# lizaibeim/mmla-audio

Measured on AMD Instinct MI355X. Metric: audio clips/sec (MFCC→logits) at 1/2/4/8 MI355X; MFCC max-abs-err vs librosa, higher is better.
Workload: dtype f16x3+f32

## Files before the change

mmla_audio_amd/csrc/context.cpp:

```cpp
#include <algorithm>
#include <cstdarg>
#include <cstdio>
#include <cstdlib>

#include "internal.h"

using namespace mmla;

namespace mmla __attribute__((visibility("hidden"))) {

int fail(mmla_ctx* c, int code, const char* fmt, ...) {
  char buf[512];
  va_list ap;
  va_start(ap, fmt);
  vsnprintf(buf, sizeof(buf), fmt, ap);
  va_end(ap);
  if (c) c->err = buf;
  return code;
}

static hipEvent_t prof_event(mmla_ctx* c) {
  if (!c->prof_pool.empty()) {
    hipEvent_t e = c->prof_pool.back();
    c->prof_pool.pop_back();
    return e;
  }
  hipEvent_t e = nullptr;
  (void)hipEventCreate(&e);
  return e;
}

int prof_begin(mmla_ctx* c, int stage) {
  if (!c->prof_on) return -1;
  ProfRec r{stage, prof_event(c), prof_event(c), 0.0};
  (void)hipEventRecord(r.a, c->stream);
  c->prof_pending.push_back(r);
  return (int)c->prof_pending.size() - 1;
}

void prof_end(mmla_ctx* c, int idx, double work) {
  if (idx < 0) return;
  ProfRec& r = c->prof_pending[idx];
  r.work = work;
  (void)hipEventRecord(r.b, c->stream);
}

int prof_collect(mmla_ctx* c) {
  for (ProfRec& r : c->prof_pending) {
    HIPCHK(c, hipEventSynchronize(r.b));
    float ms = 0.0f;
    HIPCHK(c, hipEventElapsedTime(&ms, r.a, r.b));
    c->prof_ms[r.stage] += ms;
    c->prof_work[r.stage] += r.work;
    c->prof_n[r.stage] += 1;
    c->prof_pool.push_back(r.a);
    c->prof_pool.push_back(r.b);
  }
  c->prof_pending.clear();
  return MMLA_OK;
}

constexpr size_t kGuardBytes = 4u << 20;
constexpr int kGuardByte = 0xA5;

int ws_get(mmla_ctx* c, int slot, size_t bytes, void** out) {
  if ((int)c->ws.size() <= slot) {
    c->ws.resize(slot + 1, nullptr);
    c->ws_size.resize(slot + 1, 0);
    c->ws_guard.resize(slot + 1, 0);
  }
  const char* ge = std::getenv("MMLA_WS_GUARD");
  const size_t guard = ge && ge[0] == '1' ? kGuardBytes : 0;
  if (c->ws_size[slot] < bytes || (guard && c->ws_size[slot] != bytes)) {
    if (c->ws[slot]) {
      HIPCHK(c, hipStreamSynchronize(c->stream));
      HIPCHK(c, hipFree(static_cast<char*>(c->ws[slot]) - c->ws_guard[slot]));
      c->ws[slot] = nullptr;
      c->ws_size[slot] = 0;
    }
    void* p = nullptr;
    if (c->debug_fail_allocs > 0) {
      --c->debug_fail_allocs;
      return fail(c, MMLA_E_OOM, "workspace slot %d: injected allocation failure (MMLA_DEBUG_FAIL_ALLOC)", slot);
    }
    if (hipMalloc(&p, bytes + 2 * guard) != hipSuccess) {
      (void)hipGetLastError();
      return fail(c, MMLA_E_OOM, "hipMalloc(%zu) failed for workspace slot %d", bytes, slot);
    }
    if (guard) {
      HIPCHK(c, hipMemsetAsync(p, kGuardByte, guard, c->stream));
      HIPCHK(c, hipMemsetAsync(static_cast<char*>(p) + guard + bytes, kGuardByte, guard, c->stream));
    }
    const char* pe = std::getenv("MMLA_WS_POISON");
    if (pe && pe[0])
      HIPCHK(c, hipMemsetAsync(static_cast<char*>(p) + guard, (int)std::strtol(pe, nullptr, 0) & 255,
                               bytes, c->stream));
    c->ws[slot] = static_cast<char*>(p) + guard;
    c->ws_size[slot] = bytes;
    c->ws_guard[slot] = guard;
  }
  *out = c->ws[slot];
  return MMLA_OK;
}

int ws_release(mmla_ctx* c) {
  HIPCHK(c, hipStreamSynchronize(c->stream));
  for (size_t i = 0; i < c->ws.size(); ++i)
    if (c->ws[i]) {
      HIPCHK(c, hipFree(static_cast<char*>(c->ws[i]) - c->ws_guard[i]));
      c->ws[i] = nullptr;
      c->ws_size[i] = 0;
      c->ws_guard[i] = 0;
    }
  return MMLA_OK;
}

static int ws_check_guards(mmla_ctx* c) {
  std::vector<unsigned char> h(kGuardBytes);
  for (size_t slot = 0; slot < c->ws.size(); ++slot) {
    const size_t g = c->ws_guard[slot];
    if (!c->ws[slot] || !g) continue;
    for (int side = 0; side < 2; ++side) {
      const char* d = static_cast<const char*>(c->ws[slot]) + (side ? c->ws_size[slot] : -(ptrdiff_t)g);
      HIPCHK(c, hipMemcpy(h.data(), d, g, hipMemcpyDeviceToHost));
      for (size_t i = 0; i < g; ++i)
        if (h[i] != kGuardByte)
          return fail(c, MMLA_E_HIP, "workspace slot %zu: %s guard overwritten at byte %zu", slot,
                      side ? "trailing" : "leading", side ? i : g - i);
    }
  }
  return MMLA_OK;
}

int finish(mmla_ctx* c, bool dev) {
  HIPCHK(c, hipGetLastError());
  bool guarded = false;
  for (size_t g : c->ws_guard) guarded |= g != 0;
  if (!dev || guarded) HIPCHK(c, hipStreamSynchronize(c->stream));
  if (guarded) return ws_check_guards(c);
  return MMLA_OK;
}

constexpr double kOdBytesPerClip = 3.0 * 128 * 151 * 32 * 4 + 128 * 151 * 3 + 128 * 151 * 4 +
                                   19 * 128 * 4 + 512 * 4 + 64;
constexpr double kSiBytesPerClip = 4.0 * 256 * 32 * 4 + 256 * 39 * 4 + 8 * 128 * 4 + 512 * 4 +
                                   1024 * 4 + 64;

int64_t microbatch(mmla_ctx* c, bool od) {
  const int64_t user = od ? c->od_mb : c->si_mb;
  if (user > 0) return user;
  const int64_t cap = od ? c->od_mb_cap : c->si_mb_cap;
  size_t fr = 0, tot = 0;
  if (hipMemGetInfo(&fr, &tot) != hipSuccess) {
    (void)hipGetLastError();
    return cap;
  }
  double held = 0;
  for (size_t b : c->ws_size) held += (double)b;
  int64_t fit = (int64_t)(((double)fr + held) * 0.9 / (od ? kOdBytesPerClip : kSiBytesPerClip));
  fit = fit / kMinMicrobatch * kMinMicrobatch;
  return std::max(kMinMicrobatch, std::min(cap, fit));
}

}

struct EnvSwitch {
  const char* name;
  bool mmla_ctx::*no;
  int mmla_ctx::*num;
};
static const EnvSwitch kEnvSwitches[] = {
    {"MMLA_DEBUG_FAIL_ALLOC", nullptr, &mmla_ctx::debug_fail_allocs},
    {"MMLA_NO_SIU", &mmla_ctx::siu, nullptr},
    {"MMLA_NO_SIPU", &mmla_ctx::sipu, nullptr},
    {"MMLA_NO_SIFIN", &mmla_ctx::sifin, nullptr},
    {"MMLA_NO_SIPAIR", &mmla_ctx::sipair, nullptr},
    {"MMLA_NO_SICHAIN", &mmla_ctx::sichain, nullptr},
    {"MMLA_NO_LSTM_SPLIT", &mmla_ctx::lstm_split, nullptr},
    {"MMLA_LSTM_SPLIT_MAX", nullptr, &mmla_ctx::lstm_split_max},
    {"MMLA_DEBUG_LSTM_SPIN", nullptr, &mmla_ctx::lstm_spin},
    {"MMLA_NO_SIPAD", &mmla_ctx::si_pad_feat, nullptr},
    {"MMLA_NO_ODU", &mmla_ctx::odu, nullptr},
    {"MMLA_NO_ODW", &mmla_ctx::odw, nullptr},
    {"MMLA_NO_VADW", &mmla_ctx::vadw, nullptr},
    {"MMLA_VADW", nullptr, &mmla_ctx::vadw_all},
    {"MMLA_RB_TILE", &mmla_ctx::rbs, nullptr},
    {"MMLA_NO_PIN_OUT", &mmla_ctx::pin_small, nullptr},
};

extern "C" {

int mmla_abi_version(void) { return MMLA_ABI_VERSION; }

int mmla_create(int device, mmla_ctx** out) {
  if (!out) return MMLA_E_INVALID;
  *out = nullptr;
  int ndev = 0;
  if (hipGetDeviceCount(&ndev) != hipSuccess || ndev == 0) return MMLA_E_HIP;
  if (device < 0 || device >= ndev) return MMLA_E_INVALID;
  if (hipSetDevice(device) != hipSuccess) return MMLA_E_HIP;
  mmla_ctx* c = new mmla_ctx();
  c->device = device;
  for (const EnvSwitch& s : kEnvSwitches)
    if (const char* v = std::getenv(s.name)) {
      if (s.no) c->*s.no = std::atoi(v) == 0;
      else c->*s.num = std::atoi(v);
    }
  if (hipStreamCreateWithFlags(&c->own_stream, hipStreamDefault) != hipSuccess) {
    delete c;
    return MMLA_E_HIP;
  }
  c->stream = c->own_stream;
  if (hipMalloc(&c->range_dev, 4 * sizeof(int)) != hipSuccess ||
      hipMemset(c->range_dev, 0, 4 * sizeof(int)) != hipSuccess ||
      hipHostMalloc(&c->range_host, 2 * sizeof(int), hipHostMallocDefault) != hipSuccess) {
    mmla_destroy(c);
    return MMLA_E_HIP;
  }
  if (c->pin_small) {
    const unsigned fl = hipHostMallocMapped | hipHostMallocCoherent;
    if (hipHostMalloc(reinterpret_cast<void**>(&c->range_map), 64, fl) != hipSuccess ||
        hipHostGetDevicePointer(reinterpret_cast<void**>(&c->range_map_dev), c->range_map, 0) != hipSuccess ||
        hipHostMalloc(reinterpret_cast<void**>(&c->pin_out), kPinSlots * kPinSlotBytes, fl) != hipSuccess ||
        hipHostGetDevicePointer(reinterpret_cast<void**>(&c->pin_out_dev), c->pin_out, 0) != hipSuccess ||
        hipHostMalloc(reinterpret_cast<void**>(&c->pin_in), kPinInBytes, hipHostMallocDefault) != hipSuccess) {
      mmla_destroy(c);
      return MMLA_E_HIP;
    }
    c->range_map[0] = c->range_map[1] = 0;
  }
  OdFeTables ot;
  od_fe_build_tables(&ot);
  if (!od_fe_tables_ok(ot)) {
    mmla_destroy(c);
    return MMLA_E_INVALID;
  }
  SiFeTables st;
  si_fe_build_tables(&st);
  if (!si_fe_tables_ok(st)) {
    mmla_destroy(c);
    return MMLA_E_INVALID;
  }
  if (hipMalloc(&c->od_tables, sizeof(OdFeTables)) != hipSuccess ||
      hipMalloc(&c->si_tables, sizeof(SiFeTables)) != hipSuccess ||
      hipMemcpy(c->od_tables, &ot, sizeof(ot), hipMemcpyHostToDevice) != hipSuccess ||
      hipMemcpy(c->si_tables, &st, sizeof(st), hipMemcpyHostToDevice) != hipSuccess) {
    mmla_destroy(c);
    return MMLA_E_HIP;
  }
  *out = c;
  return MMLA_OK;
}

int mmla_destroy(mmla_ctx* c) {
  if (!c) return MMLA_E_INVALID;
  (void)hipSetDevice(c->device);
  if (c->stream) (void)hipStreamSynchronize(c->stream);
  free_allocs(c->od_allocs);
  free_allocs(c->si_allocs);
  free_allocs(c->si_head_allocs);
  for (size_t i = 0; i < c->ws.size(); ++i)
    if (c->ws[i]) (void)hipFree(static_cast<char*>(c->ws[i]) - c->ws_guard[i]);
  if (c->od_tables) (void)hipFree(c->od_tables);
  if (c->si_tables) (void)hipFree(c->si_tables);
  if (c->nr_tables) (void)hipFree(c->nr_tables);
  if (c->nr_thresh) (void)hipFree(c->nr_thresh);
  if (c->range_dev) (void)hipFree(c->range_dev);
  if (c->vad_state) (void)hipFree(c->vad_state);
  if (c->cap_state) (void)hipFree(c->cap_state);
  for (void* p : c->cap_buf)
    if (p) (void)hipFree(p);
  if (c->range_host) (void)hipHostFree(c->range_host);
  if (c->range_map) (void)hipHostFree(c->range_map);
  if (c->pin_out) (void)hipHostFree(c->pin_out);
  if (c->pin_in) (void)hipHostFree(c->pin_in);
  (void)prof_collect(c);
  for (hipEvent_t e : c->prof_pool) (void)hipEventDestroy(e);
  if (c->own_stream) (void)hipStreamDestroy(c->own_stream);
  delete c;
  return MMLA_OK;
}

const char* mmla_last_error(const mmla_ctx* c) { return c ? c->err.c_str() : "null context"; }

int mmla_set_stream(mmla_ctx* c, void* s) {
  if (!c) return MMLA_E_INVALID;
  hipStream_t ns = s ? static_cast<hipStream_t>(s) : c->own_stream;
  if (ns != c->stream) {
    HIPCHK(c, hipSetDevice(c->device));
    hipEvent_t e = nullptr;
    HIPCHK(c, hipEventCreateWithFlags(&e, hipEventDisableTiming));
    const hipError_t r1 = hipEventRecord(e, c->stream);
    const hipError_t r2 = r1 == hipSuccess ? hipStreamWaitEvent(ns, e, 0) : r1;
    (void)hipEventDestroy(e);
    HIPCHK(c, r2);
  }
  c->stream = ns;
  return MMLA_OK;
}

int mmla_range_check(mmla_ctx* c, int64_t* f32_reruns) {
  if (!c) return MMLA_E_INVALID;
  HIPCHK(c, hipSetDevice(c->device));
  HIPCHK(c, hipStreamSynchronize(c->stream));
  if (f32_reruns) *f32_reruns = c->range_reruns;
  int flag = 0, timeout = 0;
  HIPCHK(c, hipMemcpy(&flag, c->range_dev, sizeof(int), hipMemcpyDeviceToHost));
  HIPCHK(c, hipMemcpy(&timeout, c->range_dev + 3, sizeof(int), hipMemcpyDeviceToHost));
  if (timeout) {
    HIPCHK(c, hipMemset(c->range_dev + 3, 0, sizeof(int)));
    return fail(c, MMLA_E_HIP,
                "a device-pointer call since the last check ran the split BiLSTM and one of its "
                "workgroups timed out waiting for the others: its probabilities are NaN; re-run it");
  }
  if (flag) {
    HIPCHK(c, hipMemset(c->range_dev, 0, sizeof(int)));
    return fail(c, MMLA_E_RANGE,
                "a device-pointer call since the last check split an operand outside the fp16 "
                "range (|x| >= 65504): its results are not valid; re-run it with MMLA_PREC_F32");
  }
  return MMLA_OK;
}

int mmla_debug_counters(mmla_ctx* c, int64_t* f32_reruns, int64_t* lstm_split_reruns) {
  if (!c) return MMLA_E_INVALID;
  if (f32_reruns) *f32_reruns = c->range_reruns;
  if (lstm_split_reruns) *lstm_split_reruns = c->lstm_split_reruns;
  return MMLA_OK;
}

int mmla_synchronize(mmla_ctx* c) { return mmla_range_check(c, nullptr); }

int mmla_get_microbatch(mmla_ctx* c, int64_t* od_clips, int64_t* si_clips) {
  if (!c) return MMLA_E_INVALID;
  HIPCHK(c, hipSetDevice(c->device));
  if (od_clips) *od_clips = microbatch(c, true);
  if (si_clips) *si_clips = microbatch(c, false);
  return MMLA_OK;
}

int mmla_release_workspace(mmla_ctx* c) {
  if (!c) return MMLA_E_INVALID;
  HIPCHK(c, hipSetDevice(c->device));
  CHK(ws_release(c));
  for (int i = 0; i < 5; ++i)
    if (c->cap_buf[i]) {
      HIPCHK(c, hipFree(c->cap_buf[i]));
      c->cap_buf[i] = nullptr;
      c->cap_bytes[i] = 0;
    }
  return MMLA_OK;
}

int mmla_set_precision(mmla_ctx* c, int mode) {
  if (!c || (mode != MMLA_PREC_F32 && mode != MMLA_PREC_F16X3)) return MMLA_E_INVALID;
  c->precision = mode;
  return MMLA_OK;
}

int mmla_set_microbatch(mmla_ctx* c, int64_t od, int64_t si) {
  if (!c || od < 0 || si < 0) return MMLA_E_INVALID;
  c->od_mb = od;
  c->si_mb = si;
  c->od_mb_cap = kOdMicrobatch;
  c->si_mb_cap = kSiMicrobatch;
  return MMLA_OK;
}

int mmla_debug_ws_slot(mmla_ctx* c, int slot, void** ptr, size_t* bytes) {
  if (!c || !ptr || !bytes || slot < 0) return MMLA_E_INVALID;
  const bool have = slot < (int)c->ws.size() && c->ws[slot];
  *ptr = have ? c->ws[slot] : nullptr;
  *bytes = have ? c->ws_size[slot] : 0;
  return MMLA_OK;
}

int mmla_profile_enable(mmla_ctx* c, int on) {
  if (!c) return MMLA_E_INVALID;
  c->prof_on = on != 0;
  return MMLA_OK;
}

int mmla_profile_read(mmla_ctx* c, double* ms, int64_t* launches, double* work, int reset) {
  if (!c) return MMLA_E_INVALID;
  CHK(prof_collect(c));
  for (int i = 0; i < MMLA_NSTAGES; ++i) {
    if (ms) ms[i] = c->prof_ms[i];
    if (launches) launches[i] = c->prof_n[i];
    if (work) work[i] = c->prof_work[i];
    if (reset) {
      c->prof_ms[i] = 0.0;
      c->prof_n[i] = 0;
      c->prof_work[i] = 0.0;
    }
  }
  return MMLA_OK;
}

}
```

mmla_audio_amd/csrc/internal.h:

```cpp
#pragma once
#include <hip/hip_runtime.h>

#include <cstdint>
#include <cstring>
#include <string>
#include <vector>

#include "../../include/mmla.h"
#include "nr.h"
#include "od_fe.h"
#include "si_fe.h"
#include "ssim.h"
#include "vad.h"

namespace mmla __attribute__((visibility("hidden"))) {

constexpr int OD_H = 128, OD_W = 151, OD_PIX = OD_H * OD_W;
constexpr int OD_IMG = OD_PIX * 3;
constexpr int SI_T = 256, SI_D = 39;
constexpr int SI_NEED_SAMPLES = 160 * 259 + 400;
constexpr int CH[9] = {32, 32, 32, 64, 64, 64, 128, 128, 128};
constexpr bool POOL[9] = {true, false, false, true, false, false, true, false, false};

struct ConvW {
  float* wt = nullptr;
  float* bias = nullptr;
  uint16_t* wh = nullptr;
  uint16_t* wl = nullptr;
  uint16_t* fh = nullptr;
  uint16_t* fl = nullptr;
  int kh = 0, kw = 0, cin = 0, cout = 0, cout_pad = 0, cin_pad = 0, kpad = 0;
  float wscale = 256.0f;
  float unscale() const { return 1.0f / (16.0f * wscale); }
};
struct BnW {
  float* scale = nullptr;
  float* shift = nullptr;
  int c = 0;
};
struct LstmW {
  float* wcat[2] = {nullptr, nullptr};
  float* bias[2] = {nullptr, nullptr};
  uint16_t* wth[2] = {nullptr, nullptr};
  uint16_t* wtl[2] = {nullptr, nullptr};
  float ws[2] = {256.0f, 256.0f};
};
struct ResUnitW {
  BnW bn_in, bn_mid;
  ConvW ca, cb, sc;
};
struct OdNet {
  ConvW stem;
  ResUnitW blk[9];
  LstmW lstm;
  float* head_w = nullptr;
  float* head_b = nullptr;
};
struct SiNet {
  ConvW stem;
  ResUnitW unit[9];
  BnW final_bn;
  LstmW lstm;
  ConvW dense;
  int k = 0, head = 0;
};

struct ProfRec {
  int stage;
  hipEvent_t a, b;
  double work;
};

constexpr int64_t kOdMicrobatch = 16384;
constexpr int64_t kSiMicrobatch = 65536;
constexpr int64_t kMinMicrobatch = 64;

constexpr size_t kPinSlotBytes = 64u << 10;
constexpr size_t kPinInBytes = 1u << 20;
constexpr int kPinSlots = 4;

}

struct mmla_ctx {
  bool prof_on = false;
  std::vector<mmla::ProfRec> prof_pending;
  std::vector<hipEvent_t> prof_pool;
  double prof_ms[MMLA_NSTAGES] = {0};
  double prof_work[MMLA_NSTAGES] = {0};
  int64_t prof_n[MMLA_NSTAGES] = {0};
  int device = 0;
  hipStream_t stream = nullptr;
  hipStream_t own_stream = nullptr;
  std::string err;
  OdFeTables* od_tables = nullptr;
  SiFeTables* si_tables = nullptr;
  bool od_loaded = false, si_loaded = false;
  mmla::OdNet od;
  mmla::SiNet si;
  std::vector<void*> od_allocs, si_allocs;
  std::vector<void*> si_head_allocs;
  std::vector<void*> ws;
  std::vector<size_t> ws_size;
  std::vector<size_t> ws_guard;
  int64_t od_mb = 0, si_mb = 0;
  int64_t od_mb_cap = mmla::kOdMicrobatch, si_mb_cap = mmla::kSiMicrobatch;
  int debug_fail_allocs = 0;
  int precision = MMLA_PREC_F16X3;
  bool siu = true;
  bool sipu = true;
  bool sifin = true;
  bool sipair = true;
  bool sichain = true;
  bool si_pad_feat = true;
  bool odu = true;
  bool odw = true;
  bool vadw = true;
  int vadw_all = 0;
  bool rbs = true;
  bool lstm_split = true;
  int lstm_split_max = 128;
  int lstm_spin = 0;
  int* range_dev = nullptr;
  int* range_host = nullptr;
  bool pin_small = true;
  int* range_map = nullptr;
  int* range_map_dev = nullptr;
  char* pin_out = nullptr;
  char* pin_out_dev = nullptr;
  char* pin_in = nullptr;
  int* range_ptr = nullptr;
  int* timeout_ptr = nullptr;
  int64_t lstm_split_reruns = 0;
  int64_t range_reruns = 0;
  bool od_f32_only = false, si_f32_only = false;
  bool loading_f16_bad = false;
  bool si_base_f16_bad = false;
  VadState* vad_state = nullptr;
  int64_t vad_streams = 0;
  int32_t* cap_state = nullptr;
  int cap_cur = 0;
  int64_t cap_streams = 0;
  int32_t cap_rate = 0, cap_channels = 0, cap_channel = 0, cap_ir = 0, cap_or = 0;
  void* cap_buf[5] = {nullptr, nullptr, nullptr, nullptr, nullptr};
  size_t cap_bytes[5] = {0, 0, 0, 0, 0};
  NrTables* nr_tables = nullptr;
  float* nr_thresh = nullptr;
  int64_t nr_profiles = 0;
  bool nr_ready = false;
  int32_t nr_bank_sr = 0;
  double ns_time_constant_s = 2.0, ns_thresh_n_mult = 2.0, ns_sigmoid_slope = 10.0;
  int32_t ns_sr = 16000;
};

namespace mmla __attribute__((visibility("hidden"))) {

int fail(mmla_ctx* c, int code, const char* fmt, ...);

#define HIPCHK(ctx, expr)                                                                        \
  do {                                                                                           \
    hipError_t e_ = (expr);                                                                      \
    if (e_ != hipSuccess)                                                                        \
      return mmla::fail(ctx, MMLA_E_HIP, "%s failed: %s (%s:%d)", #expr, hipGetErrorString(e_), \
                        __FILE__, __LINE__);                                                     \
  } while (0)

#define CHK(expr)              \
  do {                         \
    int r_ = (expr);           \
    if (r_ != MMLA_OK) return r_; \
  } while (0)

int prof_begin(mmla_ctx* c, int stage);
void prof_end(mmla_ctx* c, int idx, double work);
int prof_collect(mmla_ctx* c);

#define LAUNCH(c, st, wk, expr)                  \
  do {                                           \
    const int pi_ = mmla::prof_begin((c), (st)); \
    HIPCHK((c), (expr));                         \
    mmla::prof_end((c), pi_, (wk));              \
  } while (0)

enum Slot {
  S_PCM = 0, S_LENS, S_IMG, S_X, S_T1, S_T2, S_T3, S_SEQ, S_HOUT, S_LOGIT, S_FEAT, S_SILENT,
  S_OUT0, S_OUT1, S_OUT2, S_OUT3, S_IN,
  S_NR_S, S_NR_BITS, S_NR_FMAX, S_NR_FRAMES, S_NR_ITEMS, S_NR_Y, S_NR_ROWS,
  S_VAD_SPEECH, S_VAD_OUT, S_VAD_LENS, S_RS_TR, S_RS_WIN, S_LSTM,
  S_TRAIN,
  S_IMG2, S_GATE_Y0, S_GATE_Y1, S_SSIM,
  S_NR_PROF, S_COND_Q, S_COND_KEPT,
  S_ROOM_P, S_ROOM_A,
  S_ENROL_VAD, S_ENROL_NW
};

enum CapBuf { CB_RAW = 0, CB_FRAMES, CB_ITEM, CB_OUT, CB_LENS };

int ws_get(mmla_ctx* c, int slot, size_t bytes, void** out);
int ws_release(mmla_ctx* c);
int64_t microbatch(mmla_ctx* c, bool od);
int finish(mmla_ctx* c, bool dev);
void free_allocs(std::vector<void*>& al);
inline bool vad_use_wave(const mmla_ctx* c, int64_t n_streams) {
  return c->vadw && (c->vadw_all > 0 || vad_wave_streams(n_streams));
}
int nr_reduce_dev(mmla_ctx* c, const float* y, int64_t n_signals, int64_t stride, int64_t len, float* out,
                  const int32_t* profile = nullptr, bool nonstationary = false);

template <typename T>
int in_ptr(mmla_ctx* c, const T* user, size_t count, bool dev, int slot, const T** d) {
  *d = user;
  if (dev || !user) return MMLA_OK;
  void* p = nullptr;
  CHK(ws_get(c, slot, count * sizeof(T), &p));
  HIPCHK(c, hipMemcpyAsync(p, user, count * sizeof(T), hipMemcpyHostToDevice, c->stream));
  *d = static_cast<const T*>(p);
  return MMLA_OK;
}

template <typename T>
int out_ptr(mmla_ctx* c, T* user, int64_t off, size_t count, bool dev, int slot, T** d) {
  if (!user) {
    *d = nullptr;
    return MMLA_OK;
  }
  if (dev) {
    *d = user + off;
    return MMLA_OK;
  }
  if (c->pin_small && c->pin_out_dev && slot >= S_OUT0 && slot < S_OUT0 + kPinSlots &&
      count * sizeof(T) <= kPinSlotBytes) {
    *d = reinterpret_cast<T*>(c->pin_out_dev + (size_t)(slot - S_OUT0) * kPinSlotBytes);
    return MMLA_OK;
  }
  void* p = nullptr;
  CHK(ws_get(c, slot, count * sizeof(T), &p));
  *d = static_cast<T*>(p);
  return MMLA_OK;
}

template <typename T>
int copy_back(mmla_ctx* c, T* user, int64_t off, const T* d, size_t count, bool dev) {
  if (!user || dev) return MMLA_OK;
  const char* dc = reinterpret_cast<const char*>(d);
  if (c->pin_out_dev && dc >= c->pin_out_dev && dc < c->pin_out_dev + kPinSlots * kPinSlotBytes) {
    HIPCHK(c, hipStreamSynchronize(c->stream));
    std::memcpy(user + off, c->pin_out + (dc - c->pin_out_dev), count * sizeof(T));
    return MMLA_OK;
  }
  HIPCHK(c, hipMemcpyAsync(user + off, d, count * sizeof(T), hipMemcpyDeviceToHost, c->stream));
  return MMLA_OK;
}


struct OdGate {
  const int32_t* lens = nullptr;
  int clip_len = -1;
  uint8_t* silent = nullptr;
  const float* ssim = nullptr;
  float ssim_threshold = 0.0f;
};

int run_od_net(mmla_ctx* c, const uint8_t* img_u8, const float* img_f32, int64_t n, float* probs,
               int32_t* argmax, OdGate gate = OdGate(), int stop = -1, const float** tap = nullptr,
               int64_t* tap_n = nullptr);
int run_si_net(mmla_ctx* c, const float* x, int64_t n, float* probs, int32_t* argmax,
               const uint8_t* silent, int ldx = SI_D, const float** tap = nullptr);

}
```

mmla_audio_amd/csrc/net_runners.cpp:

```cpp
#include <algorithm>

#include "conv.h"
#include "conv_h3.h"
#include "internal.h"
#include "nets.h"
#include "odu.h"
#include "resblk.h"
#include "siu.h"

using namespace mmla;

namespace {

ConvArgs conv_args(const ConvW& w, const float* x, float* y, int n, int h, int wd, int stride,
                   const BnW* bn, int pro, int epi, const float* res) {
  ConvArgs a{};
  a.x = x;
  a.wt = w.wt;
  a.bias = w.bias;
  a.scale = bn ? bn->scale : nullptr;
  a.shift = bn ? bn->shift : nullptr;
  a.res = res;
  a.y = y;
  a.n = n;
  a.h = h;
  a.w = wd;
  a.cin = w.cin;
  a.ho = (h + stride - 1) / stride;
  a.wo = (wd + stride - 1) / stride;
  a.cout = w.cout;
  a.cout_pad = w.cout_pad;
  a.ldy = w.cout;
  a.kh = w.kh;
  a.kw = w.kw;
  a.stride = stride;
  const int th = std::max((a.ho - 1) * stride + w.kh - h, 0);
  const int tw = std::max((a.wo - 1) * stride + w.kw - wd, 0);
  a.pad_h = th / 2;
  a.pad_w = tw / 2;
  a.pro = pro;
  a.epi = epi;
  return a;
}

double conv_flops(const ConvArgs& a) {
  return 2.0 * (double)a.n * a.ho * a.wo * a.kh * a.kw * a.cin * a.cout;
}

int conv_run(mmla_ctx* c, const ConvArgs& a, int stage = MMLA_STAGE_CONV) {
  LAUNCH(c, stage, conv_flops(a), conv_launch(a, c->stream));
  return MMLA_OK;
}

ConvH3Args conv_h3_args(const ConvW& w, const float* x, float* y, int n, int h, int wd, const BnW* bn,
                        int pro, int epi, const float* res, int* range_flag) {
  ConvH3Args a{};
  a.x = x;
  a.wh = w.wh;
  a.wl = w.wl;
  a.unscale = w.unscale();
  a.bias = w.bias;
  a.scale = bn ? bn->scale : nullptr;
  a.shift = bn ? bn->shift : nullptr;
  a.res = res;
  a.y = y;
  a.n = n;
  a.h = h;
  a.w = wd;
  a.cin = w.cin;
  a.cin_pad = w.cin_pad;
  a.cout = w.cout;
  a.cout_pad = w.cout_pad;
  a.kh = w.kh;
  a.kw = w.kw;
  a.pad_h = (w.kh - 1) / 2;
  a.pad_w = (w.kw - 1) / 2;
  a.pro = pro;
  a.epi = epi;
  a.range_flag = range_flag;
  return a;
}

int conv_spatial(mmla_ctx* c, const ConvW& w, const float* x, float* y, int n, int h, int wd,
                 const BnW* bn, int pro, int epi, const float* res, bool pool_out = false,
                 int pool_in_h = 0, const ConvW* sc = nullptr, const float* sc_x = nullptr,
                 int sc_h = 0) {
  if (c->precision == MMLA_PREC_F16X3 && w.wh) {
    ConvH3Args a = conv_h3_args(w, x, y, n, h, wd, bn, pro, epi, res, c->range_ptr);
    double sc_flops = 0.0;
    if (sc && sc_x) {
      a.sc_x = sc_x;
      a.sc_wh = sc->wh;
      a.sc_wl = sc->wl;
      a.sc_bias = sc->bias;
      a.sc_cin = sc->cin;
      a.sc_h = sc_h;
      a.sc_unscale = sc->unscale();
      sc_flops = sc_h > 0 ? 2.0 * n * h * sc->cin * sc->cout
                          : 2.0 * n * ((h + 1) / 2) * ((wd + 1) / 2) * sc->cin * sc->cout;
    }
    a.pool_in = pool_in_h > 0;
    a.h_in = pool_in_h;
    a.pool_out = pool_out ? 1 : 0;
    LAUNCH(c, MMLA_STAGE_CONV, 2.0 * n * h * wd * w.kh * w.kw * w.cin * w.cout + sc_flops,
           conv_h3_launch(a, c->stream));
    return MMLA_OK;
  }
  ConvArgs a = conv_args(w, x, y, n, h, wd, 1, bn, pro, epi, res);
  if (!pool_out) return conv_run(c, a);
  return fail(c, MMLA_E_INVALID, "pooled epilogue needs the 3xFP16 conv path");
}

int ws_floats(mmla_ctx* c, int slot, size_t count, float** out) {
  void* p = nullptr;
  CHK(ws_get(c, slot, count * sizeof(float), &p));
  *out = static_cast<float*>(p);
  return MMLA_OK;
}

double lstm_flops(int64_t n, int T, int D) { return 2.0 * n * T * 2 * (256.0 + D) * 1024.0; }

hipError_t lstm_run(mmla_ctx* c, const LstmW& L, const float* seq, int64_t n, int T, float* out) {
  if (c->precision == MMLA_PREC_F16X3 && L.wth[0] && c->lstm_split &&
      n <= std::min(c->lstm_split_max, bilstm_h3_split_max_clips())) {
    void* ws = nullptr;
    if (ws_get(c, S_LSTM, bilstm_h3_split_ws_bytes(), &ws) != MMLA_OK) return hipErrorOutOfMemory;
    return bilstm_h3_split_launch(seq, (int)n, T, 128, L.wth[0], L.wtl[0], L.wth[1], L.wtl[1],
                                  L.bias[0], L.bias[1], out, c->range_ptr, L.ws[0], L.ws[1], ws,
                                  c->timeout_ptr, c->lstm_spin, c->stream);
  }
  if (c->precision == MMLA_PREC_F16X3 && L.wth[0])
    return bilstm_h3_launch(seq, (int)n, T, 128, L.wth[0], L.wtl[0], L.wth[1], L.wtl[1], L.bias[0],
                            L.bias[1], out, c->range_ptr, L.ws[0], L.ws[1], c->stream);
  return bilstm_launch(seq, (int)n, T, 128, L.wcat[0], L.wcat[1], L.bias[0], L.bias[1], out,
                       c->stream);
}


enum OdPath {
  OD_STRIPS,
  OD_TILES,
  OD_ODU,
  OD_PAIR
};
struct OdChoice {
  OdPath path;
  bool stem;
  int strips;
};

bool strips_ok(const ResUnitW& B, bool pool, int h, int w) {
  return B.ca.wh && B.cb.wh && (!pool || B.sc.wh) && B.ca.cin_pad == B.ca.cin && B.ca.cout_pad == 32 &&
         B.cb.cin_pad == 32 && B.cb.cout_pad == 32 && B.cb.kh == 4 && B.cb.kw == 1 &&
         (!pool || (B.sc.cin_pad == B.ca.cin && B.sc.cout_pad == 32)) &&
         rbs_supported(h, w, B.ca.cin, B.ca.cout, pool);
}

bool tiles_ok(const ResUnitW& B, bool pool) {
  return B.ca.fh && B.cb.fh && B.cb.kpad == 4 * B.cb.cin && (!pool || B.sc.fh) &&
         resblk_supported(B.ca.cin, B.ca.cout, pool);
}

bool odu_ok(const ResUnitW& B, bool pool, int h, int w) {
  return B.ca.wh && B.cb.wh && (!pool || B.sc.wh) && odu_supported(h, w, B.ca.cin, B.ca.cout, pool) &&
         B.ca.cin_pad == B.ca.cin && B.ca.cout_pad == B.ca.cout && B.cb.cin == B.ca.cout &&
         B.cb.cout == B.ca.cout && B.cb.cin_pad == B.cb.cin && B.cb.cout_pad == B.cb.cout &&
         B.cb.kh == 4 && B.cb.kw == 1 &&
         (!pool || (B.sc.cin == B.ca.cin && B.sc.cout == B.ca.cout && B.sc.cout_pad == B.sc.cout));
}

OdChoice od_choose(const mmla_ctx* c, const ResUnitW& B, int b, int h, int w, int stop) {
  OdChoice k{OD_PAIR, false, 1};
  if (c->precision != MMLA_PREC_F16X3) return k;
  if (c->rbs && strips_ok(B, POOL[b], h, w)) k.path = OD_STRIPS;
  else if (tiles_ok(B, POOL[b])) k.path = OD_TILES;
  else if (c->odu && odu_ok(B, POOL[b], h, w)) {
    k.path = OD_ODU;
    k.strips = c->odw && odu_two_strips(h, w, B.ca.cin, B.ca.cout, POOL[b]) ? 2 : 1;
  }
  k.stem = b == 0 && stop != 0 && (k.path == OD_STRIPS || k.path == OD_TILES);
  return k;
}

ResBlkArgs resblk_args(const ResUnitW& B, bool pool, bool fused, const float* x, float* y, int64_t n,
                       int h, int w, int* range_flag, const ConvW* stem, const uint8_t* img_u8,
                       const float* img_f32) {
  ResBlkArgs r{};
  r.x = x;
  r.y = y;
  r.w1h = fused ? B.ca.fh : B.ca.wh;
  r.w1l = fused ? B.ca.fl : B.ca.wl;
  r.b1 = B.ca.bias;
  r.u1 = B.ca.unscale();
  r.s1 = B.bn_in.scale;
  r.t1 = B.bn_in.shift;
  r.w2h = fused ? B.cb.fh : B.cb.wh;
  r.w2l = fused ? B.cb.fl : B.cb.wl;
  r.b2 = B.cb.bias;
  r.u2 = B.cb.unscale();
  r.s2 = B.bn_mid.scale;
  r.t2 = B.bn_mid.shift;
  if (pool) {
    r.wsh = fused ? B.sc.fh : B.sc.wh;
    r.wsl = fused ? B.sc.fl : B.sc.wl;
    r.bs = B.sc.bias;
    r.us = B.sc.unscale();
  }
  if (stem) {
    r.x = nullptr;
    r.img8 = img_u8;
    r.imgf = img_u8 ? nullptr : img_f32;
    r.wst = stem->wt;
    r.bst = stem->bias;
    r.ldst = stem->cout_pad;
  }
  r.n = (int)n;
  r.h = h;
  r.w = w;
  r.range_flag = range_flag;
  return r;
}

OduArgs odu_args(const ResUnitW& B, bool pool, const float* x, float* y, int64_t n, int* range_flag) {
  OduArgs o{};
  o.x = x;
  o.y = y;
  o.wah = B.ca.wh;
  o.wal = B.ca.wl;
  o.wbh = B.cb.wh;
  o.wbl = B.cb.wl;
  o.ba = B.ca.bias;
  o.bb = B.cb.bias;
  o.s_in = B.bn_in.scale;
  o.t_in = B.bn_in.shift;
  o.s_mid = B.bn_mid.scale;
  o.t_mid = B.bn_mid.shift;
  o.ua = B.ca.unscale();
  o.ub = B.cb.unscale();
  o.n = (int)n;
  o.range_flag = range_flag;
  if (pool) {
    o.wsh = B.sc.wh;
    o.wsl = B.sc.wl;
    o.bs = B.sc.bias;
    o.us = B.sc.unscale();
  }
  return o;
}

double od_block_flops(const ResUnitW& B, bool pool, int64_t n, int h, int w) {
  return 2.0 * n * h * w * (9.0 * B.ca.cin * B.ca.cout + 4.0 * B.cb.cin * B.cb.cout) +
         (pool ? 2.0 * n * ((h + 1) / 2) * ((w + 1) / 2) * B.sc.cin * B.sc.cout : 0.0);
}

int od_block_pair(mmla_ctx* c, const ResUnitW& B, bool pool, int n, int h, int w, float* X, float*& T1,
                  float*& T2, float** out) {
  CHK(conv_spatial(c, B.ca, X, T1, n, h, w, &B.bn_in, PRO_BN_ELU, EPI_BIAS, nullptr));
  if (!pool) {
    *out = X;
    return conv_spatial(c, B.cb, T1, X, n, h, w, &B.bn_mid, PRO_BN_ELU, EPI_ADD, X);
  }
  if (c->precision != MMLA_PREC_F16X3) {
    CHK(conv_spatial(c, B.cb, T1, T2, n, h, w, &B.bn_mid, PRO_BN_ELU, EPI_BIAS, nullptr));
    ConvArgs s = conv_args(B.sc, X, T1, n, h, w, 2, nullptr, PRO_NONE, EPI_ADD_POOL, T2);
    s.hp = h;
    s.wp = w;
    CHK(conv_run(c, s));
  } else if (B.sc.wh && B.sc.cout == B.cb.cout && B.cb.cout_pad == B.sc.cout_pad) {
    CHK(conv_spatial(c, B.cb, T1, T2, n, h, w, &B.bn_mid, PRO_BN_ELU, EPI_BIAS, nullptr, true, 0, &B.sc,
                     X));
    std::swap(T1, T2);
  } else {
    CHK(conv_spatial(c, B.cb, T1, T2, n, h, w, &B.bn_mid, PRO_BN_ELU, EPI_BIAS, nullptr, true));
    CHK(conv_run(c, conv_args(B.sc, X, T1, n, h, w, 2, nullptr, PRO_NONE, EPI_ADD, T2)));
  }
  *out = T1;
  return MMLA_OK;
}

}

namespace mmla __attribute__((visibility("hidden"))) {

int run_od_net(mmla_ctx* c, const uint8_t* img_u8, const float* img_f32, int64_t n, float* probs,
               int32_t* argmax, OdGate gate, int stop, const float** tap, int64_t* tap_n) {
  const OdNet& W = c->od;
  const size_t big = (size_t)n * OD_PIX * 32;
  float *X, *T1, *T2, *SEQ, *H;
  CHK(ws_floats(c, S_X, big, &X));
  CHK(ws_floats(c, S_T1, big, &T1));
  CHK(ws_floats(c, S_T2, big, &T2));
  CHK(ws_floats(c, S_SEQ, (size_t)n * 19 * 128, &SEQ));
  CHK(ws_floats(c, S_HOUT, (size_t)n * 512, &H));
  const double stem_flops = 2.0 * n * OD_PIX * 3 * 16;
  const OdChoice first = od_choose(c, W.blk[0], 0, OD_H, OD_W, stop);
  if (!first.stem)
    LAUNCH(c, MMLA_STAGE_GLUE, stem_flops,
           od_stem_launch(img_u8, img_f32, n * OD_PIX, W.stem.cout_pad, W.stem.wt, W.stem.bias, X,
                          c->stream));
  int h = OD_H, w = OD_W;
  if (stop == 0) {
    *tap = X;
    *tap_n = n * OD_PIX * 16;
    return MMLA_OK;
  }
  for (int b = 0; b < 9; ++b) {
    const ResUnitW& B = W.blk[b];
    const bool pool = POOL[b];
    const OdChoice k = b == 0 ? first : od_choose(c, B, b, h, w, stop);
    const double flops = od_block_flops(B, pool, n, h, w) + (k.stem ? stem_flops : 0.0);
    float* out = T1;
    switch (k.path) {
      case OD_STRIPS:
      case OD_TILES: {
        const bool tiles = k.path == OD_TILES;
        const ResBlkArgs r = resblk_args(B, pool, tiles, X, T1, n, h, w, c->range_ptr,
                                         k.stem ? &W.stem : nullptr, img_u8, img_f32);
        LAUNCH(c, MMLA_STAGE_CONV, flops,
               tiles ? resblk_launch(r, B.ca.cin, B.ca.cout, pool, c->stream)
                     : rbs_launch(r, B.ca.cin, B.ca.cout, pool, c->stream));
        break;
      }
      case OD_ODU: {
        const OduArgs o = odu_args(B, pool, X, T1, n, c->range_ptr);
        LAUNCH(c, MMLA_STAGE_CONV, flops,
               odu_launch(o, h, w, B.ca.cin, B.ca.cout, pool, k.strips, c->stream));
        break;
      }
      case OD_PAIR:
        CHK(od_block_pair(c, B, pool, (int)n, h, w, X, T1, T2, &out));
        break;
    }
    if (pool) {
      h = (h + 1) / 2;
      w = (w + 1) / 2;
    }
    if (out != X) std::swap(X, T1);
    if (stop == b + 1) {
      *tap = X;
      *tap_n = n * h * w * CH[b];
      return MMLA_OK;
    }
  }
  LAUNCH(c, MMLA_STAGE_GLUE, (double)n * h * w * 128,
         mean_h_launch(X, (int)n, h, w, 128, SEQ, c->stream));
  if (stop == 10) {
    *tap = SEQ;
    *tap_n = n * w * 128;
    return MMLA_OK;
  }
  LAUNCH(c, MMLA_STAGE_LSTM, lstm_flops(n, w, 128),
         lstm_run(c, W.lstm, SEQ, n, w, H));
  if (stop == 11) {
    *tap = H;
    *tap_n = n * 512;
    return MMLA_OK;
  }
  LAUNCH(c, MMLA_STAGE_HEAD, 2.0 * n * 512 * 2,
         od_head_launch(H, (int)n, W.head_w, W.head_b, probs, argmax,
                        gate.lens, gate.clip_len, gate.silent, gate.ssim, gate.ssim_threshold,
                        c->stream));
  return MMLA_OK;
}

}


namespace {

bool siu_ok(const ResUnitW& U, int cin) {
  return U.ca.wh && U.cb.wh && siu_chain_supported(cin, cin, false, 1, false) && U.ca.cin == cin &&
         U.ca.cout == cin && U.cb.cin == cin && U.cb.cout == cin && U.ca.cin_pad == cin && U.ca.cout_pad == cin &&
         U.cb.cout_pad == cin;
}

bool sipu_ok(const ResUnitW& U, int cin) {
  return U.ca.wh && U.cb.wh && U.sc.wh && siu_chain_supported(cin, U.ca.cout, true, 1, false) &&
         U.ca.cin_pad == cin && U.ca.cout_pad == U.ca.cout && U.cb.cin == U.ca.cout && U.cb.cout == U.ca.cout &&
         U.cb.cout_pad == U.ca.cout && U.sc.cin == cin && U.sc.cout == U.ca.cout &&
         U.sc.cout_pad == U.ca.cout;
}

int si_choose(const mmla_ctx* c, const SiNet& W, int u) {
  if (!c->siu || c->precision != MMLA_PREC_F16X3) return 0;
  const int cin = W.unit[u].ca.cin, C = W.unit[u].ca.cout;
  auto plain = [&](int v) { return v < 9 && !POOL[v] && siu_ok(W.unit[v], C); };
  if (POOL[u]) {
    if (!c->sipu || !sipu_ok(W.unit[u], cin)) return 0;
    return c->sichain && siu_chain_supported(cin, C, true, 3, false) && plain(u + 1) && plain(u + 2) ? 3 : 1;
  }
  if (!siu_ok(W.unit[u], cin)) return 0;
  return c->sipair && siu_chain_supported(cin, cin, false, 2, false) && plain(u + 1) ? 2 : 1;
}

double si_unit_flops(const ResUnitW& U, bool pool, int64_t n, int t) {
  return 2.0 * n * t *
         (3.0 * U.ca.cin * U.ca.cout + 3.0 * U.cb.cin * U.cb.cout + (pool ? 1.0 * U.sc.cin * U.sc.cout : 0.0));
}

SiuArgs siu_args(const ResUnitW& U, const float* x, float* y, int64_t n, int t, int* range_flag,
                 int t_src = 0) {
  SiuArgs s{};
  s.n = (int)n;
  s.t = t;
  s.range_flag = range_flag;
  s.x = x;
  s.y = y;
  s.wah = U.ca.wh;
  s.wal = U.ca.wl;
  s.wbh = U.cb.wh;
  s.wbl = U.cb.wl;
  s.ba = U.ca.bias;
  s.bb = U.cb.bias;
  s.s_in = U.bn_in.scale;
  s.t_in = U.bn_in.shift;
  s.s_mid = U.bn_mid.scale;
  s.t_mid = U.bn_mid.shift;
  s.ua = U.ca.unscale();
  s.ub = U.cb.unscale();
  if (t_src > 0) {
    s.t_src = t_src;
    s.wsh = U.sc.wh;
    s.wsl = U.sc.wl;
    s.bs = U.sc.bias;
    s.us = U.sc.unscale();
  }
  return s;
}

}

namespace mmla __attribute__((visibility("hidden"))) {

int run_si_net(mmla_ctx* c, const float* x, int64_t n, float* probs, int32_t* argmax,
               const uint8_t* silent, int ldx, const float** tap) {
  const SiNet& W = c->si;
  const size_t big = (size_t)n * SI_T * 32;
  float *X, *T1, *XP, *R, *SEQ, *H, *L;
  CHK(ws_floats(c, S_X, big, &X));
  CHK(ws_floats(c, S_T1, big, &T1));
  CHK(ws_floats(c, S_T2, big, &XP));
  CHK(ws_floats(c, S_T3, big, &R));
  CHK(ws_floats(c, S_SEQ, (size_t)n * 8 * 128, &SEQ));
  CHK(ws_floats(c, S_HOUT, (size_t)n * 512, &H));
  CHK(ws_floats(c, S_LOGIT, (size_t)n * W.dense.cout_pad, &L));
  int t = SI_T;
  const bool h3 = c->precision == MMLA_PREC_F16X3;
  bool fused_final = false;
  ConvW stem = W.stem;
  if (ldx == SI_D + 1 && h3 && stem.wh && stem.cin_pad > SI_D) stem.cin = ldx;
  else if (ldx != SI_D) return fail(c, MMLA_E_INVALID, "padded SI features need the 3xFP16 stem");
  CHK(conv_spatial(c, stem, x, X, (int)n, t, 1, nullptr, PRO_NONE, EPI_BIAS, nullptr));
  for (int u = 0; u < 9; ++u) {
    const ResUnitW& U = W.unit[u];
    const int cin = U.ca.cin;
    const bool pool = POOL[u];
    const int tp = pool ? (t + 1) / 2 : t;
    const int units = si_choose(c, W, u);
    float* out = R;
    if (units > 0) {
      const int C = U.ca.cout;
      SiuArgs s[3];
      double flops = 0.0;
      for (int k = 0; k < units; ++k) {
        const bool first = k == 0;
        s[k] = siu_args(W.unit[u + k], first ? X : nullptr, k == units - 1 ? R : nullptr, n, tp, c->range_ptr,
                        first && pool ? t : 0);
        flops += si_unit_flops(W.unit[u + k], first && pool, n, tp);
      }
      if (u + units == 9 && c->sifin && tp % 4 == 0 && siu_chain_supported(cin, C, pool, units, true)) {
        SiuArgs& last = s[units - 1];
        last.y = nullptr;
        last.seq = SEQ;
        last.fs = W.final_bn.scale;
        last.ft = W.final_bn.shift;
        fused_final = true;
      }
      LAUNCH(c, MMLA_STAGE_CONV, flops, siu_chain_launch(s, units, pool, cin, C, c->stream));
      u += units - 1;
    } else if (pool) {
      if (h3 && U.ca.wh) {
        CHK(conv_spatial(c, U.ca, X, T1, (int)n, tp, 1, &U.bn_in, PRO_BN_RELU, EPI_BIAS, nullptr,
                         false, t));
      } else {
        LAUNCH(c, MMLA_STAGE_GLUE, (double)n * t * cin,
               maxpool_t2_launch(X, (int)n, t, cin, XP, c->stream));
        CHK(conv_spatial(c, U.ca, XP, T1, (int)n, tp, 1, &U.bn_in, PRO_BN_RELU, EPI_BIAS, nullptr));
      }
      if (h3 && U.cb.wh && U.sc.wh && U.sc.cout == U.cb.cout && U.sc.cout_pad == U.cb.cout_pad) {
        CHK(conv_spatial(c, U.cb, T1, R, (int)n, tp, 1, &U.bn_mid, PRO_BN_RELU, EPI_ADD, nullptr, false,
                         0, &U.sc, X, t));
      } else {
        CHK(conv_run(c, conv_args(U.sc, X, R, (int)n, t, 1, 2, nullptr, PRO_NONE, EPI_BIAS, nullptr)));
        CHK(conv_spatial(c, U.cb, T1, R, (int)n, tp, 1, &U.bn_mid, PRO_BN_RELU, EPI_ADD, R));
      }
    } else {
      CHK(conv_spatial(c, U.ca, X, T1, (int)n, t, 1, &U.bn_in, PRO_BN_RELU, EPI_BIAS, nullptr));
      CHK(conv_spatial(c, U.cb, T1, X, (int)n, t, 1, &U.bn_mid, PRO_BN_RELU, EPI_ADD, X));
      out = X;
    }
    if (out != X) std::swap(X, R);
    t = tp;
  }
  if (!fused_final)
    LAUNCH(c, MMLA_STAGE_GLUE, 3.0 * n * t * 128,
           bn_relu_avgpool4_launch(X, (int)n, t, 128, W.final_bn.scale, W.final_bn.shift,
                                   SEQ, c->stream));
  LAUNCH(c, MMLA_STAGE_LSTM, lstm_flops(n, t / 4, 128),
         lstm_run(c, W.lstm, SEQ, n, t / 4, H));
  if (tap) {
    *tap = H;
    return MMLA_OK;
  }
  if (h3 && W.dense.wh && W.dense.cin % 32 == 0) {
    ConvH3Args a = conv_h3_args(W.dense, H, L, (int)n, 1, 1, nullptr, PRO_NONE, EPI_BIAS, nullptr,
                                c->range_ptr);
    a.cout = W.dense.cout_pad;
    LAUNCH(c, MMLA_STAGE_HEAD, 2.0 * n * W.dense.cin * W.dense.cout, conv_h3_launch(a, c->stream));
  } else {
    ConvArgs d = conv_args(W.dense, H, L, (int)n, 1, 1, 1,
                           nullptr, PRO_NONE, EPI_BIAS, nullptr);
    d.ldy = W.dense.cout_pad;
    CHK(conv_run(c, d, MMLA_STAGE_HEAD));
  }
  LAUNCH(c, MMLA_STAGE_HEAD, 4.0 * n * W.k,
         si_head_launch(L, (int)n, W.k, W.dense.cout_pad, W.head, probs,
                        argmax, silent, c->stream));
  return MMLA_OK;
}

}
```

mmla_audio_amd/csrc/rbs.hip:

```cpp
#include "f16x3.h"
#include "resblk.h"

namespace {

constexpr int NT = 256;
constexpr int TW = 16;
constexpr int R = 8;
constexpr int C = 32;
#ifndef RBS_TRACE
#define RBS_TRACE 0
#endif
#if RBS_TRACE
__device__ unsigned long long rbs_trace_buf[2048 * 4 * 4 * 8];
#define RBS_T(i) do { if (bid < 2048 && k >= 2 && k < 6) tt[i] = __builtin_amdgcn_s_memtime(); } while (0)
#define RBS_TFLUSH() do { if (bid < 2048 && k >= 2 && k < 6 && lane == 0) { for (int i_ = 0; i_ < 8; ++i_) rbs_trace_buf[(((size_t)bid * 4 + wave) * 4 + (k - 2)) * 8 + i_] = tt[i_]; } } while (0)
#else
#define RBS_T(i) do { } while (0)
#define RBS_TFLUSH() do { } while (0)
#endif

template <int H, int W, int CIN, bool POOL>
struct SG {
  static constexpr int XW = TW + 2;
  static constexpr int XRING = R + 2, TRING = R + 3;
  static constexpr int XROW = XW * CIN;
  static constexpr int XPLANE = XRING * XROW;
  static constexpr int TROW = TW * C;
  static constexpr int TPLANE = TRING * TROW;
  static constexpr int NCHUNK = H / R;
  static constexpr int STRIPS = (W + TW - 1) / TW;
  static constexpr int QPP = CIN / 4;
  static constexpr int MAXT = (R * XW * QPP + NT - 1) / NT;
  static constexpr int MAXT0 = (4 * XW * QPP + NT - 1) / NT;
  static constexpr int KPT = CIN / 16;
  static constexpr int KS1 = 9 * KPT, KS2 = 8;
  static constexpr bool W2L = CIN == 16;
  static constexpr int MINB = CIN == 16 ? 3 : 2;
  static constexpr int PF = 3;
  static constexpr int PD = CIN == 16 ? 1 : 2;
  static_assert(H % R == 0, "geometry");
  static_assert(NT % QPP == 0, "a thread's channel quad is fixed");
  static_assert(XROW <= 1024 && W * CIN * 4 < 65536 && W * 12 < 65536, "staging task fields");
};

template <int CIN>
MMLA_DEV int xoff(int slot, int x, int g) {
  constexpr int XROW = (TW + 2) * CIN;
  const int f = CIN == 32 ? ((x >> 1) & 3) : ((x >> 1) & 1);
  return slot * XROW + x * CIN + 8 * (g ^ f);
}
template <bool POOL>
MMLA_DEV int toff(int slot, int j, int c, int g) {
  const int f = POOL ? (((c >> 2) ^ (2 * (j & 1))) & 3) : ((c >> 2) & 3);
  return slot * (TW * C) + c * C + 8 * (g ^ f);
}

template <int H, int W, int CIN, bool POOL, bool STEM>
__global__ void __launch_bounds__(NT, (SG<H, W, CIN, POOL>::MINB)) rbs_kernel(ResBlkArgs a) {
  using G = SG<H, W, CIN, POOL>;
  static_assert(!STEM || (CIN == 16 && POOL), "the stem feeds block 1");
  static_assert(POOL || CIN == C, "residual blocks keep their width");
  __shared__ __attribute__((aligned(16))) _Float16 sx[2 * G::XPLANE];
  __shared__ __attribute__((aligned(16))) _Float16 st[2 * G::TPLANE];
  __shared__ float4 spar[3 * C / 4 + (STEM ? 16 : 0)];
  __shared__ __attribute__((aligned(16))) _Float16 sw2[G::W2L ? 2 * G::KS2 * 512 : 8];

  const int tid = threadIdx.x, lane = tid & 63;
  const int wave = __builtin_amdgcn_readfirstlane(tid >> 6);
  const int h = lane >> 5;
  const uint32_t bid = xcd_block_id();
  const int clip = (int)(bid / G::STRIPS);
  const int w0 = (int)(bid - (uint32_t)clip * G::STRIPS) * TW;
  const int lofs = lane * 8;
  float rmax = 0.0f;

  float* const sp = reinterpret_cast<float*>(spar);
  if (tid < C) {
    const float s2 = a.s2[tid];
    sp[tid] = 16.0f * (s2 * a.u1);
    sp[C + tid] = 16.0f * fmaf(a.b1[tid], s2, a.t2[tid]);
    sp[2 * C + tid] = a.b2[tid];
  }
  if constexpr (STEM) {
    if (tid < 64) {
      const int co = tid >> 2, k = tid & 3;
      sp[3 * C + tid] = k < 3 ? a.wst[k * a.ldst + co] : a.bst[co];
    }
  }
  const __amdgpu_buffer_rsrc_t rw1h = w_rsrc(a.w1h), rw1l = w_rsrc(a.w1l);
  f16x8 w2h[G::W2L ? 1 : G::KS2], w2l[G::W2L ? 1 : G::KS2];
  if constexpr (G::W2L) {
    for (int e = tid; e < 2 * G::KS2 * 64; e += NT) {
      const int pl = e / (G::KS2 * 64), i = e - pl * (G::KS2 * 64);
      *reinterpret_cast<f16x8*>(sw2 + 8 * e) = *reinterpret_cast<const f16x8*>((pl ? a.w2l : a.w2h) + 8 * i);
    }
  } else {
    const __amdgpu_buffer_rsrc_t rw2h = w_rsrc(a.w2h), rw2l = w_rsrc(a.w2l);
#pragma unroll
    for (int s = 0; s < G::KS2; ++s) {
      w2h[s] = w_frag(rw2h, s * 512, lofs);
      w2l[s] = w_frag(rw2l, s * 512, lofs);
    }
  }
  f16x8 wsh_, wsl_;
  if constexpr (POOL) {
    wsh_ = w_frag(w_rsrc(a.wsh), 0, lofs);
    wsl_ = w_frag(w_rsrc(a.wsl), 0, lofs);
  }
  const int q = tid % G::QPP;
  float bnw[4][4];
  __syncthreads();
#pragma unroll
  for (int c = 0; c < 4; ++c) {
    const float s16 = 16.0f * a.s1[4 * q + c], t16 = 16.0f * a.t1[4 * q + c];
    if constexpr (STEM) {
      const float4 v = spar[3 * C / 4 + 4 * q + c];
      bnw[c][0] = s16 * v.x;
      bnw[c][1] = s16 * v.y;
      bnw[c][2] = s16 * v.z;
      bnw[c][3] = fmaf(s16, v.w, t16);
    } else {
      bnw[c][0] = s16;
      bnw[c][1] = t16;
    }
  }

  constexpr uint32_t ROWB = STEM ? 0u : (uint32_t)W * CIN * 4;
  const __amdgpu_buffer_rsrc_t rx = STEM ? w_rsrc(nullptr) :
      __builtin_amdgcn_make_buffer_rsrc(const_cast<float*>(a.x) + (int64_t)clip * H * W * CIN, (short)0,
                                        (int)(H * ROWB), 0x00020000);
  const bool im8 = STEM && a.img8 != nullptr;
  const __amdgpu_buffer_rsrc_t rimg = !STEM ? w_rsrc(nullptr) :
      __builtin_amdgcn_make_buffer_rsrc(im8 ? (void*)(a.img8 + (int64_t)clip * H * W * 3)
                                            : (void*)(a.imgf + (int64_t)clip * H * W * 3),
                                        (short)0, (int)(H * W * 3 * (im8 ? 1 : 4)), 0x00020000);
  uint32_t tinfo[G::MAXT];
#pragma unroll
  for (int j = 0; j < G::MAXT; ++j) {
    const int t = tid + j * NT;
    const int px = t / G::QPP;
    const int rr = px / G::XW, x = px - rr * G::XW;
    const int iw = w0 - 1 + x;
    const bool col_ok = iw >= 0 && iw < W;
    const uint32_t tc = !col_ok ? 0u : STEM ? (uint32_t)iw * (a.img8 ? 3u : 12u) : (uint32_t)(iw * CIN + 4 * q) * 4u;
    tinfo[j] = (uint32_t)(xoff<CIN>(0, x, q >> 1) + 4 * (q & 1)) | ((uint32_t)(rr & 15) << 10) |
               ((uint32_t)col_ok << 14) | ((uint32_t)(rr < R) << 15) | (tc << 16);
  }
  auto load_src = [&](int ih, int iw, bool col_ok) -> float4 {
    if constexpr (STEM) {
      const int pix = ih * W + iw;
      const bool ok = col_ok && ih >= 0 && ih < H;
      if (im8) {
        const uint32_t off = ok ? (uint32_t)pix * 3u : 0x80000000u;
        const uint32_t r = __builtin_amdgcn_raw_buffer_load_b8(rimg, off, 0, 0);
        const uint32_t g = __builtin_amdgcn_raw_buffer_load_b8(rimg, off + 1u, 0, 0);
        const uint32_t b = __builtin_amdgcn_raw_buffer_load_b8(rimg, off + 2u, 0, 0);
        return make_float4(__builtin_bit_cast(float, r), __builtin_bit_cast(float, g), __builtin_bit_cast(float, b), 0.f);
      }
      const uint32_t off = ok ? (uint32_t)pix * 12u : 0x80000000u;
      return make_float4(__builtin_bit_cast(float, __builtin_amdgcn_raw_buffer_load_b32(rimg, off, 0, 0)),
                         __builtin_bit_cast(float, __builtin_amdgcn_raw_buffer_load_b32(rimg, off + 4u, 0, 0)),
                         __builtin_bit_cast(float, __builtin_amdgcn_raw_buffer_load_b32(rimg, off + 8u, 0, 0)), 0.f);
    } else {
      const uint32_t off = col_ok ? (uint32_t)ih * ROWB + (uint32_t)(iw * CIN + 4 * q) * 4u : 0x80000000u;
      return __builtin_bit_cast(float4, __builtin_amdgcn_raw_buffer_load_b128(rx, off, 0, 0));
    }
  };
  auto img_px = [&](float4 v) -> float4 {
    if (im8)
      return make_float4((float)__builtin_bit_cast(uint32_t, v.x), (float)__builtin_bit_cast(uint32_t, v.y),
                         (float)__builtin_bit_cast(uint32_t, v.z), 0.f);
    return v;
  };
  auto load_task = [&](int r0, int j) -> float4 {
    const uint32_t ti = tinfo[j];
    const uint32_t off = (ti >> 14) & 1u ? (uint32_t)((r0 + (int)((ti >> 10) & 15)) * (STEM ? W * 3 * (im8 ? 1 : 4) : (int)ROWB)) + (ti >> 16)
                                         : 0x80000000u;
    if constexpr (STEM) {
      if (im8) {
        const uint32_t r = __builtin_amdgcn_raw_buffer_load_b8(rimg, off, 0, 0);
        const uint32_t g = __builtin_amdgcn_raw_buffer_load_b8(rimg, off + 1u, 0, 0);
        const uint32_t b = __builtin_amdgcn_raw_buffer_load_b8(rimg, off + 2u, 0, 0);
        return make_float4(__builtin_bit_cast(float, r), __builtin_bit_cast(float, g), __builtin_bit_cast(float, b), 0.f);
      }
      return make_float4(__builtin_bit_cast(float, __builtin_amdgcn_raw_buffer_load_b32(rimg, off, 0, 0)),
                         __builtin_bit_cast(float, __builtin_amdgcn_raw_buffer_load_b32(rimg, off + 4u, 0, 0)),
                         __builtin_bit_cast(float, __builtin_amdgcn_raw_buffer_load_b32(rimg, off + 8u, 0, 0)), 0.f);
    } else {
      return __builtin_bit_cast(float4, __builtin_amdgcn_raw_buffer_load_b128(rx, off, 0, 0));
    }
  };
  auto stage4 = [&](int o, bool in, float4 v, auto MASK_) {
    constexpr bool MASK = decltype(MASK_)::value;
    if constexpr (STEM) v = img_px(v);
    float u[4];
#pragma unroll
    for (int c = 0; c < 4; ++c) {
      if constexpr (STEM) {
        float acc = v.x * bnw[c][0];
        acc = fmaf(v.y, bnw[c][1], acc);
        acc = fmaf(v.z, bnw[c][2], acc);
        u[c] = acc + bnw[c][3];
      } else {
        u[c] = fmaf((&v.x)[c], bnw[c][0], bnw[c][1]);
      }
    }
    float e[4];
#pragma unroll
    for (int c = 0; c < 4; ++c) e[c] = (!MASK || in) ? elu16(u[c]) : 0.0f;
    rmax = fmaxf(rmax, amax4(e[0], e[1], e[2], e[3]));
    f16x4 hv, lv;
    split4(e[0], e[1], e[2], e[3], hv, lv);
    *reinterpret_cast<f16x4*>(sx + o) = hv;
    *reinterpret_cast<f16x4*>(sx + G::XPLANE + o) = lv;
  };
  auto stage_task = [&](int r0, int j, float4 v, auto MASK_) {
    const uint32_t ti = tinfo[j];
    if (((ti >> 14) & 3u) != 3u) return;
    const int rr = (int)((ti >> 10) & 15);
    uint32_t slot = (uint32_t)((r0 + 1) % G::XRING) + (uint32_t)rr;
    slot = min(slot, slot - (uint32_t)G::XRING);
    stage4((int)slot * G::XROW + (int)(ti & 1023), r0 + rr < H, v, MASK_);
  };
  for (int e = tid; e < 2 * G::XRING * G::XW * G::QPP; e += NT) {
    const int pl = e / (G::XRING * G::XW * G::QPP), r = e - pl * (G::XRING * G::XW * G::QPP);
    const int slot = r / (G::XW * G::QPP), x = (r / G::QPP) % G::XW, qq = r % G::QPP;
    const int iw = w0 - 1 + x;
    if (iw < 0 || iw >= W)
      *reinterpret_cast<f16x4*>(sx + pl * G::XPLANE + xoff<CIN>(slot, x, qq >> 1) + 4 * (qq & 1)) = f16x4{};
  }
  const int n = lane & 31, nr = n >> 4, nc = n & 15;
  int xco[3][G::KPT];
#pragma unroll
  for (int dx = 0; dx < 3; ++dx)
#pragma unroll
    for (int ks = 0; ks < G::KPT; ++ks) xco[dx][ks] = xoff<CIN>(0, nc + dx, G::KPT == 2 ? 2 * ks + h : h);

  f16x8 w1h[G::PF], w1l[G::PF];
  auto gemm1_issue = [&]() {
#pragma unroll
    for (int s = 0; s < G::PF; ++s) {
      w1h[s] = w_frag(rw1h, s * 512, lofs);
      w1l[s] = w_frag(rw1l, s * 512, lofs);
    }
  };
  auto gemm1 = [&](int j0) -> f32x16 {
    f32x16 acc;
#pragma unroll
    for (int i = 0; i < 16; ++i) acc[i] = 0.0f;
    int xr[3];
#pragma unroll
    for (int dy = 0; dy < 3; ++dy) {
      const uint32_t sl = (uint32_t)(j0 % G::XRING) + (uint32_t)(nr + dy);
      xr[dy] = (int)min(sl, sl - (uint32_t)G::XRING) * G::XROW;
    }
    auto xo = [&](int s) {
      const int tap = s / G::KPT, ks = s % G::KPT;
      return xr[tap / 3] + xco[tap % 3][ks];
    };
    f16x8 nxh = *reinterpret_cast<const f16x8*>(sx + xo(0));
    f16x8 nxl = *reinterpret_cast<const f16x8*>(sx + G::XPLANE + xo(0));
#pragma unroll
    for (int s = 0; s < G::KS1; ++s) {
      const f16x8 bh = w1h[s % G::PF], bl = w1l[s % G::PF];
      if (s + G::PF < G::KS1) {
        w1h[s % G::PF] = w_frag(rw1h, (s + G::PF) * 512, lofs);
        w1l[s % G::PF] = w_frag(rw1l, (s + G::PF) * 512, lofs);
      }
      const f16x8 xh = nxh, xl = nxl;
      if (s + 1 < G::KS1) {
        nxh = *reinterpret_cast<const f16x8*>(sx + xo(s + 1));
        nxl = *reinterpret_cast<const f16x8*>(sx + G::XPLANE + xo(s + 1));
      }
      acc = __builtin_amdgcn_mfma_f32_32x32x16_f16(bl, xh, acc, 0, 0, 0);
      acc = __builtin_amdgcn_mfma_f32_32x32x16_f16(bh, xl, acc, 0, 0, 0);
      acc = __builtin_amdgcn_mfma_f32_32x32x16_f16(bh, xh, acc, 0, 0, 0);
      __builtin_amdgcn_sched_barrier(0);
    }
    return acc;
  };
  auto t1_write = [&](int j0, const f32x16& acc) {
    const int j = j0 + nr;
    const uint32_t sl = (uint32_t)((j0 + 1) % G::TRING) + (uint32_t)nr;
    const int slot = (int)min(sl, sl - (uint32_t)G::TRING);
    if (j0 < H) {
#pragma unroll
      for (int jj = 0; jj < 4; ++jj) {
        const int c0 = 8 * jj + 4 * h;
        const float4 sv = spar[c0 / 4], cv = spar[C / 4 + c0 / 4];
        float e[4];
        e[0] = elu16(fmaf(acc[4 * jj + 0], sv.x, cv.x));
        e[1] = elu16(fmaf(acc[4 * jj + 1], sv.y, cv.y));
        e[2] = elu16(fmaf(acc[4 * jj + 2], sv.z, cv.z));
        e[3] = elu16(fmaf(acc[4 * jj + 3], sv.w, cv.w));
        rmax = fmaxf(rmax, amax4(e[0], e[1], e[2], e[3]));
        f16x4 hv, lv;
        split4(e[0], e[1], e[2], e[3], hv, lv);
        const int o = toff<POOL>(slot, j, nc, jj) + 4 * h;
        *reinterpret_cast<f16x4*>(st + o) = hv;
        *reinterpret_cast<f16x4*>(st + G::TPLANE + o) = lv;
      }
    } else {
#pragma unroll
      for (int jj = 0; jj < 4; ++jj) {
        const int o = toff<POOL>(slot, j, nc, jj) + 4 * h;
        *reinterpret_cast<f16x4*>(st + o) = f16x4{};
        *reinterpret_cast<f16x4*>(st + G::TPLANE + o) = f16x4{};
      }
    }
  };

  {
    constexpr int T0 = 4 * G::XW * G::QPP;
#pragma unroll
    for (int j = 0; j < G::MAXT0; ++j) {
      const int t = tid + j * NT;
      const int px = t / G::QPP;
      const int rr = px / G::XW, x = px - rr * G::XW;
      const int ih = rr - 1, iw = w0 - 1 + x;
      const bool col_ok = iw >= 0 && iw < W;
      const float4 v = load_src(ih, iw, col_ok);
      if (t < T0 && col_ok)
        stage4(xoff<CIN>((ih + 1) % G::XRING, x, q >> 1) + 4 * (q & 1), ih >= 0, v, std::true_type{});
    }
    for (int e = tid; e < 2 * G::TROW / 8; e += NT)
      *reinterpret_cast<f16x8*>(st + (e >= G::TROW / 8 ? G::TPLANE - G::TROW : 0) + 8 * e) = f16x8{};
  }
  __syncthreads();
  if (wave == 0) {
    gemm1_issue();
    const f32x16 acc = gemm1(0);
    t1_write(0, acc);
  }
  float4 preA[G::MAXT], preB[G::PD == 2 ? G::MAXT : 1];
#pragma unroll
  for (int j = 0; j < G::MAXT; ++j) preA[j] = load_task(3, j);
  if constexpr (G::PD == 2) {
#pragma unroll
    for (int j = 0; j < G::MAXT; ++j) preB[j] = load_task(3 + R, j);
  }
  __syncthreads();

  const int win = n >> 2;
  const int sc_col = w0 + 2 * win;
  float bsc = 0.0f;
  if constexpr (POOL) bsc = a.bs[n];

#if RBS_TRACE
  unsigned long long tt[8];
#endif
  static_assert(G::NCHUNK % 2 == 0, "chunk pairs");
  auto chunk = [&](const int k, float4* pre) {
    RBS_T(0);
    const int rx0 = R * k + 3;
    const int j0 = R * k + 2 + 2 * wave;
    const int o0 = R * k + 2 * wave;
    if (k + 1 < G::NCHUNK) {
#pragma unroll
      for (int j = 0; j < G::MAXT; ++j) stage_task(rx0, j, pre[j], std::false_type{});
    } else {
#pragma unroll
      for (int j = 0; j < G::MAXT; ++j) stage_task(rx0, j, pre[j], std::true_type{});
    }
    gemm1_issue();
    RBS_T(1);
    __syncthreads();
    RBS_T(2);
    {
      const f32x16 acc = gemm1(j0);
      RBS_T(3);
      t1_write(j0, acc);
    }
    RBS_T(4);
    const int pr = POOL ? (n & 3) >> 1 : nr;
    const int pc = POOL ? 2 * (n >> 2) + (n & 1) : nc;
    float4 rsd[POOL ? 1 : 4];
    float4 scpx = make_float4(0.f, 0.f, 0.f, 0.f);
    if constexpr (!POOL) {
      const uint32_t off = w0 + pc < W ? (uint32_t)(o0 + pr) * ROWB + (uint32_t)((w0 + pc) * C + 4 * h) * 4u : 0x80000000u;
#pragma unroll
      for (int jj = 0; jj < 4; ++jj)
        rsd[jj] = __builtin_bit_cast(float4, __builtin_amdgcn_raw_buffer_load_b128(rx, off, jj * 32, 0));
    } else {
      scpx = load_src(o0, sc_col, sc_col < W);
    }
    if (k + G::PD < G::NCHUNK) {
#pragma unroll
      for (int j = 0; j < G::MAXT; ++j) pre[j] = load_task(rx0 + G::PD * R, j);
    }
    __syncthreads();
    RBS_T(5);
    f32x16 acc;
#pragma unroll
    for (int i = 0; i < 16; ++i) acc[i] = 0.0f;
    {
      int tr[4], tj[4];
#pragma unroll
      for (int dy = 0; dy < 4; ++dy) {
        tj[dy] = o0 + pr - 1 + dy;
        const uint32_t sl = (uint32_t)(o0 % G::TRING) + (uint32_t)(pr + dy);
        tr[dy] = (int)min(sl, sl - (uint32_t)G::TRING);
      }
      auto to = [&](int s) { return toff<POOL>(tr[s >> 1], tj[s >> 1], pc, 2 * (s & 1) + h); };
      auto step2 = [&](f16x8 xh, f16x8 xl, f16x8 gh, f16x8 gl) {
        if constexpr (POOL) {
          acc = __builtin_amdgcn_mfma_f32_32x32x16_f16(xh, gl, acc, 0, 0, 0);
          acc = __builtin_amdgcn_mfma_f32_32x32x16_f16(xl, gh, acc, 0, 0, 0);
          acc = __builtin_amdgcn_mfma_f32_32x32x16_f16(xh, gh, acc, 0, 0, 0);
        } else {
          acc = __builtin_amdgcn_mfma_f32_32x32x16_f16(gl, xh, acc, 0, 0, 0);
          acc = __builtin_amdgcn_mfma_f32_32x32x16_f16(gh, xl, acc, 0, 0, 0);
          acc = __builtin_amdgcn_mfma_f32_32x32x16_f16(gh, xh, acc, 0, 0, 0);
        }
      };
      if constexpr (G::W2L) {
        f16x8 fxh[2], fxl[2], fgh[2], fgl[2];
        auto fetch = [&](int s) {
          fxh[s & 1] = *reinterpret_cast<const f16x8*>(st + to(s));
          fxl[s & 1] = *reinterpret_cast<const f16x8*>(st + G::TPLANE + to(s));
          fgh[s & 1] = *reinterpret_cast<const f16x8*>(sw2 + s * 512 + lofs);
          fgl[s & 1] = *reinterpret_cast<const f16x8*>(sw2 + (G::KS2 + s) * 512 + lofs);
        };
        fetch(0);
#pragma unroll
        for (int s = 0; s < G::KS2; ++s) {
          if (s + 1 < G::KS2) fetch(s + 1);
          step2(fxh[s & 1], fxl[s & 1], fgh[s & 1], fgl[s & 1]);
          if (s + 1 < G::KS2) pin_group<1, 4>(); else pin_group<1, 0>();
        }
      } else {
        f16x8 nxh = *reinterpret_cast<const f16x8*>(st + to(0));
        f16x8 nxl = *reinterpret_cast<const f16x8*>(st + G::TPLANE + to(0));
#pragma unroll
        for (int s = 0; s < G::KS2; ++s) {
          const f16x8 xh = nxh, xl = nxl;
          if (s + 1 < G::KS2) {
            nxh = *reinterpret_cast<const f16x8*>(st + to(s + 1));
            nxl = *reinterpret_cast<const f16x8*>(st + G::TPLANE + to(s + 1));
          }
          step2(xh, xl, w2h[s], w2l[s]);
          __builtin_amdgcn_sched_barrier(0);
        }
      }
    }
    RBS_T(6);
    if constexpr (!POOL) {
      const int ow = w0 + pc, oh = o0 + pr;
      if (ow < W) {
#pragma unroll
        for (int jj = 0; jj < 4; ++jj) {
          const int c0 = 8 * jj + 4 * h;
          const float4 b = spar[2 * C / 4 + c0 / 4];
          const float4 r = rsd[jj];
          const float4 v = make_float4(fmaf(acc[4 * jj + 0], a.u2, b.x) + r.x, fmaf(acc[4 * jj + 1], a.u2, b.y) + r.y,
                                       fmaf(acc[4 * jj + 2], a.u2, b.z) + r.z, fmaf(acc[4 * jj + 3], a.u2, b.w) + r.w);
          *reinterpret_cast<float4*>(a.y + (((int64_t)clip * H + oh) * W + ow) * C + c0) = v;
        }
      }
    } else {
      f32x16 sacc;
#pragma unroll
      for (int i = 0; i < 16; ++i) sacc[i] = 0.0f;
      {
        float o8[8];
        const float4 px = img_px(scpx);
#pragma unroll
        for (int c = 0; c < 8; ++c) {
          const float4 wv = spar[3 * C / 4 + 8 * h + c];
          float s = px.x * wv.x;
          s = fmaf(px.y, wv.y, s);
          s = fmaf(px.z, wv.z, s);
          o8[c] = sc_col < W ? 16.0f * (s + wv.w) : 0.0f;
        }
        rmax = fmaxf(rmax, fmaxf(amax4(o8[0], o8[1], o8[2], o8[3]), amax4(o8[4], o8[5], o8[6], o8[7])));
        f16x4 h0, l0, h1, l1;
        split4(o8[0], o8[1], o8[2], o8[3], h0, l0);
        split4(o8[4], o8[5], o8[6], o8[7], h1, l1);
        const f16x8 ah = {h0[0], h0[1], h0[2], h0[3], h1[0], h1[1], h1[2], h1[3]};
        const f16x8 al = {l0[0], l0[1], l0[2], l0[3], l1[0], l1[1], l1[2], l1[3]};
        sacc = __builtin_amdgcn_mfma_f32_32x32x16_f16(ah, wsl_, sacc, 0, 0, 0);
        sacc = __builtin_amdgcn_mfma_f32_32x32x16_f16(al, wsh_, sacc, 0, 0, 0);
        sacc = __builtin_amdgcn_mfma_f32_32x32x16_f16(ah, wsh_, sacc, 0, 0, 0);
      }
      constexpr int HP = H / 2, WP = (W + 1) / 2;
      const int co = n;
      const float b2 = sp[2 * C + co], bs = bsc;
      const int prow = (R / 2) * k + wave;
#pragma unroll
      for (int jj = 0; jj < 4; ++jj) {
        const int wdw = 2 * jj + h;
        const int cc = w0 + 2 * wdw;
        if (cc >= W) continue;
        float m0 = fmaf(acc[4 * jj + 0], a.u2, b2);
        float m1 = fmaf(acc[4 * jj + 1], a.u2, b2);
        float m2 = fmaf(acc[4 * jj + 2], a.u2, b2);
        float m3 = fmaf(acc[4 * jj + 3], a.u2, b2);
        if (cc + 1 >= W) {
          m1 = m0;
          m3 = m2;
        }
        const float mx = fmaxf(fmaxf(m0, m1), fmaxf(m2, m3)) + fmaf(sacc[4 * jj], a.us, bs);
        a.y[(((int64_t)clip * HP + prow) * WP + (w0 >> 1) + wdw) * C + co] = mx;
      }
    }
    RBS_T(7);
    RBS_TFLUSH();
  };
  if constexpr (G::PD == 2) {
#pragma unroll 1
    for (int k = 0; k < G::NCHUNK; k += 2) {
      chunk(k, preA);
      chunk(k + 1, preB);
    }
  } else {
#pragma unroll 1
    for (int k = 0; k < G::NCHUNK; ++k) chunk(k, preA);
  }
  if (!(rmax < SPLIT_MAX) && a.range_flag) *a.range_flag = 1;
}

template <int H, int W, int CIN, bool POOL, bool STEM>
hipError_t launch(const ResBlkArgs& a, hipStream_t s) {
  using G = SG<H, W, CIN, POOL>;
  const int64_t blocks = (int64_t)a.n * G::STRIPS;
  if (blocks > 0x7fffffffLL) return hipErrorInvalidValue;
  hipLaunchKernelGGL((rbs_kernel<H, W, CIN, POOL, STEM>), dim3((unsigned)blocks), dim3(NT), 0, s, a);
  return hipGetLastError();
}

}

#if RBS_TRACE
extern "C" int mmla_debug_rbs_trace(unsigned long long* out) {
  return hipMemcpyFromSymbol(out, HIP_SYMBOL(rbs_trace_buf), sizeof(rbs_trace_buf)) == hipSuccess ? 0 : -2;
}
#endif

bool rbs_supported(int h, int w, int cin, int c, bool pool) {
  return c == 32 && ((h == 128 && w == 151 && cin == 16 && pool) || (h == 64 && w == 76 && cin == 32 && !pool));
}

hipError_t rbs_launch(const ResBlkArgs& a, int cin, int c, bool pool, hipStream_t s) {
  if (a.n == 0) return hipSuccess;
  if (!rbs_supported(a.h, a.w, cin, c, pool) || !a.y || !a.w1h || !a.w1l || !a.w2h || !a.w2l)
    return hipErrorInvalidValue;
  if (pool) {
    if (!a.wsh || !a.wsl || !a.bs) return hipErrorInvalidValue;
    if (a.img8 || a.imgf) return launch<128, 151, 16, true, true>(a, s);
    return hipErrorInvalidValue;
  }
  if (!a.x || a.x == a.y) return hipErrorInvalidValue;
  return launch<64, 76, 32, false, false>(a, s);
}
```

mmla_audio_amd/csrc/resblk.h:

```cpp
#pragma once
#include <hip/hip_runtime.h>
#include <stdint.h>

struct ResBlkArgs {
  const float* x;
  const uint16_t* w1h;
  const uint16_t* w1l;
  const float* b1;
  const float* s1;
  const float* t1;
  const uint16_t* w2h;
  const uint16_t* w2l;
  const float* b2;
  const float* s2;
  const float* t2;
  const uint16_t* wsh;
  const uint16_t* wsl;
  const float* bs;
  const uint8_t* img8;
  const float* imgf;
  const float* wst;
  const float* bst;
  int ldst;
  float* y;
  int n, h, w;
  int tiles_h, tiles_w;
  int* range_flag;
  float u1, u2, us;
};

int resblk_k1pad(int cin);
bool resblk_supported(int cin, int c, bool pool);
hipError_t resblk_launch(ResBlkArgs a, int cin, int c, bool pool, hipStream_t stream);
void resblk_split_weights(const float* w, int taps, int cin, int cout, int kpad, uint16_t* hi,
                          uint16_t* lo, bool frag, float wscale);

bool rbs_supported(int h, int w, int cin, int c, bool pool);
hipError_t rbs_launch(const ResBlkArgs& a, int cin, int c, bool pool, hipStream_t stream);
```

Baseline: 169,500.

## Add LDS-staged first-conv weight variant of strip resblock kernel

```diff
diff --git a/mmla_audio_amd/csrc/context.cpp b/mmla_audio_amd/csrc/context.cpp
--- a/mmla_audio_amd/csrc/context.cpp
+++ b/mmla_audio_amd/csrc/context.cpp
@@ -185,6 +185,7 @@
     {"MMLA_NO_VADW", &mmla_ctx::vadw, nullptr},
     {"MMLA_VADW", nullptr, &mmla_ctx::vadw_all},
     {"MMLA_RB_TILE", &mmla_ctx::rbs, nullptr},
+    {"MMLA_NO_RBS_W1L", &mmla_ctx::rbs_w1l, nullptr},
     {"MMLA_NO_PIN_OUT", &mmla_ctx::pin_small, nullptr},
 };
 
diff --git a/mmla_audio_amd/csrc/internal.h b/mmla_audio_amd/csrc/internal.h
--- a/mmla_audio_amd/csrc/internal.h
+++ b/mmla_audio_amd/csrc/internal.h
@@ -117,6 +117,7 @@
   bool vadw = true;
   int vadw_all = 0;
   bool rbs = true;
+  bool rbs_w1l = true;
   bool lstm_split = true;
   int lstm_split_max = 128;
   int lstm_spin = 0;
diff --git a/mmla_audio_amd/csrc/net_runners.cpp b/mmla_audio_amd/csrc/net_runners.cpp
--- a/mmla_audio_amd/csrc/net_runners.cpp
+++ b/mmla_audio_amd/csrc/net_runners.cpp
@@ -147,6 +147,7 @@
   OdPath path;
   bool stem;
   int strips;
+  bool w1_lds;
 };
 
 bool strips_ok(const ResUnitW& B, bool pool, int h, int w) {
@@ -170,11 +171,14 @@
 }
 
 OdChoice od_choose(const mmla_ctx* c, const ResUnitW& B, int b, int h, int w, int stop) {
-  OdChoice k{OD_PAIR, false, 1};
+  OdChoice k{OD_PAIR, false, 1, false};
   if (c->precision != MMLA_PREC_F16X3) return k;
-  if (c->rbs && strips_ok(B, POOL[b], h, w)) k.path = OD_STRIPS;
-  else if (tiles_ok(B, POOL[b])) k.path = OD_TILES;
-  else if (c->odu && odu_ok(B, POOL[b], h, w)) {
+  if (c->rbs && strips_ok(B, POOL[b], h, w)) {
+    k.path = OD_STRIPS;
+    k.w1_lds = c->rbs_w1l && !POOL[b];
+  } else if (tiles_ok(B, POOL[b])) {
+    k.path = OD_TILES;
+  } else if (c->odu && odu_ok(B, POOL[b], h, w)) {
     k.path = OD_ODU;
     k.strips = c->odw && odu_two_strips(h, w, B.ca.cin, B.ca.cout, POOL[b]) ? 2 : 1;
   }
@@ -318,7 +322,7 @@
                                          k.stem ? &W.stem : nullptr, img_u8, img_f32);
         LAUNCH(c, MMLA_STAGE_CONV, flops,
                tiles ? resblk_launch(r, B.ca.cin, B.ca.cout, pool, c->stream)
-                     : rbs_launch(r, B.ca.cin, B.ca.cout, pool, c->stream));
+                     : rbs_launch(r, B.ca.cin, B.ca.cout, pool, k.w1_lds, c->stream));
         break;
       }
       case OD_ODU: {
diff --git a/mmla_audio_amd/csrc/rbs.hip b/mmla_audio_amd/csrc/rbs.hip
--- a/mmla_audio_amd/csrc/rbs.hip
+++ b/mmla_audio_amd/csrc/rbs.hip
@@ -1,523 +1,8 @@
-#include "f16x3.h"
-#include "resblk.h"
+#define RBS_KERNEL rbs_kernel
+#define RBS_W1L false
+#include "rbs_body.h"
 
 namespace {
-
-constexpr int NT = 256;
-constexpr int TW = 16;
-constexpr int R = 8;
-constexpr int C = 32;
-#ifndef RBS_TRACE
-#define RBS_TRACE 0
-#endif
-#if RBS_TRACE
-__device__ unsigned long long rbs_trace_buf[2048 * 4 * 4 * 8];
-#define RBS_T(i) do { if (bid < 2048 && k >= 2 && k < 6) tt[i] = __builtin_amdgcn_s_memtime(); } while (0)
-#define RBS_TFLUSH() do { if (bid < 2048 && k >= 2 && k < 6 && lane == 0) { for (int i_ = 0; i_ < 8; ++i_) rbs_trace_buf[(((size_t)bid * 4 + wave) * 4 + (k - 2)) * 8 + i_] = tt[i_]; } } while (0)
-#else
-#define RBS_T(i) do { } while (0)
-#define RBS_TFLUSH() do { } while (0)
-#endif
-
-template <int H, int W, int CIN, bool POOL>
-struct SG {
-  static constexpr int XW = TW + 2;
-  static constexpr int XRING = R + 2, TRING = R + 3;
-  static constexpr int XROW = XW * CIN;
-  static constexpr int XPLANE = XRING * XROW;
-  static constexpr int TROW = TW * C;
-  static constexpr int TPLANE = TRING * TROW;
-  static constexpr int NCHUNK = H / R;
-  static constexpr int STRIPS = (W + TW - 1) / TW;
-  static constexpr int QPP = CIN / 4;
-  static constexpr int MAXT = (R * XW * QPP + NT - 1) / NT;
-  static constexpr int MAXT0 = (4 * XW * QPP + NT - 1) / NT;
-  static constexpr int KPT = CIN / 16;
-  static constexpr int KS1 = 9 * KPT, KS2 = 8;
-  static constexpr bool W2L = CIN == 16;
-  static constexpr int MINB = CIN == 16 ? 3 : 2;
-  static constexpr int PF = 3;
-  static constexpr int PD = CIN == 16 ? 1 : 2;
-  static_assert(H % R == 0, "geometry");
-  static_assert(NT % QPP == 0, "a thread's channel quad is fixed");
-  static_assert(XROW <= 1024 && W * CIN * 4 < 65536 && W * 12 < 65536, "staging task fields");
-};
-
-template <int CIN>
-MMLA_DEV int xoff(int slot, int x, int g) {
-  constexpr int XROW = (TW + 2) * CIN;
-  const int f = CIN == 32 ? ((x >> 1) & 3) : ((x >> 1) & 1);
-  return slot * XROW + x * CIN + 8 * (g ^ f);
-}
-template <bool POOL>
-MMLA_DEV int toff(int slot, int j, int c, int g) {
-  const int f = POOL ? (((c >> 2) ^ (2 * (j & 1))) & 3) : ((c >> 2) & 3);
-  return slot * (TW * C) + c * C + 8 * (g ^ f);
-}
-
-template <int H, int W, int CIN, bool POOL, bool STEM>
-__global__ void __launch_bounds__(NT, (SG<H, W, CIN, POOL>::MINB)) rbs_kernel(ResBlkArgs a) {
-  using G = SG<H, W, CIN, POOL>;
-  static_assert(!STEM || (CIN == 16 && POOL), "the stem feeds block 1");
-  static_assert(POOL || CIN == C, "residual blocks keep their width");
-  __shared__ __attribute__((aligned(16))) _Float16 sx[2 * G::XPLANE];
-  __shared__ __attribute__((aligned(16))) _Float16 st[2 * G::TPLANE];
-  __shared__ float4 spar[3 * C / 4 + (STEM ? 16 : 0)];
-  __shared__ __attribute__((aligned(16))) _Float16 sw2[G::W2L ? 2 * G::KS2 * 512 : 8];
-
-  const int tid = threadIdx.x, lane = tid & 63;
-  const int wave = __builtin_amdgcn_readfirstlane(tid >> 6);
-  const int h = lane >> 5;
-  const uint32_t bid = xcd_block_id();
-  const int clip = (int)(bid / G::STRIPS);
-  const int w0 = (int)(bid - (uint32_t)clip * G::STRIPS) * TW;
-  const int lofs = lane * 8;
-  float rmax = 0.0f;
-
-  float* const sp = reinterpret_cast<float*>(spar);
-  if (tid < C) {
-    const float s2 = a.s2[tid];
-    sp[tid] = 16.0f * (s2 * a.u1);
-    sp[C + tid] = 16.0f * fmaf(a.b1[tid], s2, a.t2[tid]);
-    sp[2 * C + tid] = a.b2[tid];
-  }
-  if constexpr (STEM) {
-    if (tid < 64) {
-      const int co = tid >> 2, k = tid & 3;
-      sp[3 * C + tid] = k < 3 ? a.wst[k * a.ldst + co] : a.bst[co];
-    }
-  }
-  const __amdgpu_buffer_rsrc_t rw1h = w_rsrc(a.w1h), rw1l = w_rsrc(a.w1l);
-  f16x8 w2h[G::W2L ? 1 : G::KS2], w2l[G::W2L ? 1 : G::KS2];
-  if constexpr (G::W2L) {
-    for (int e = tid; e < 2 * G::KS2 * 64; e += NT) {
-      const int pl = e / (G::KS2 * 64), i = e - pl * (G::KS2 * 64);
-      *reinterpret_cast<f16x8*>(sw2 + 8 * e) = *reinterpret_cast<const f16x8*>((pl ? a.w2l : a.w2h) + 8 * i);
-    }
-  } else {
-    const __amdgpu_buffer_rsrc_t rw2h = w_rsrc(a.w2h), rw2l = w_rsrc(a.w2l);
-#pragma unroll
-    for (int s = 0; s < G::KS2; ++s) {
-      w2h[s] = w_frag(rw2h, s * 512, lofs);
-      w2l[s] = w_frag(rw2l, s * 512, lofs);
-    }
-  }
-  f16x8 wsh_, wsl_;
-  if constexpr (POOL) {
-    wsh_ = w_frag(w_rsrc(a.wsh), 0, lofs);
-    wsl_ = w_frag(w_rsrc(a.wsl), 0, lofs);
-  }
-  const int q = tid % G::QPP;
-  float bnw[4][4];
-  __syncthreads();
-#pragma unroll
-  for (int c = 0; c < 4; ++c) {
-    const float s16 = 16.0f * a.s1[4 * q + c], t16 = 16.0f * a.t1[4 * q + c];
-    if constexpr (STEM) {
-      const float4 v = spar[3 * C / 4 + 4 * q + c];
-      bnw[c][0] = s16 * v.x;
-      bnw[c][1] = s16 * v.y;
-      bnw[c][2] = s16 * v.z;
-      bnw[c][3] = fmaf(s16, v.w, t16);
-    } else {
-      bnw[c][0] = s16;
-      bnw[c][1] = t16;
-    }
-  }
-
-  constexpr uint32_t ROWB = STEM ? 0u : (uint32_t)W * CIN * 4;
-  const __amdgpu_buffer_rsrc_t rx = STEM ? w_rsrc(nullptr) :
-      __builtin_amdgcn_make_buffer_rsrc(const_cast<float*>(a.x) + (int64_t)clip * H * W * CIN, (short)0,
-                                        (int)(H * ROWB), 0x00020000);
-  const bool im8 = STEM && a.img8 != nullptr;
-  const __amdgpu_buffer_rsrc_t rimg = !STEM ? w_rsrc(nullptr) :
-      __builtin_amdgcn_make_buffer_rsrc(im8 ? (void*)(a.img8 + (int64_t)clip * H * W * 3)
-                                            : (void*)(a.imgf + (int64_t)clip * H * W * 3),
-                                        (short)0, (int)(H * W * 3 * (im8 ? 1 : 4)), 0x00020000);
-  uint32_t tinfo[G::MAXT];
-#pragma unroll
-  for (int j = 0; j < G::MAXT; ++j) {
-    const int t = tid + j * NT;
-    const int px = t / G::QPP;
-    const int rr = px / G::XW, x = px - rr * G::XW;
-    const int iw = w0 - 1 + x;
-    const bool col_ok = iw >= 0 && iw < W;
-    const uint32_t tc = !col_ok ? 0u : STEM ? (uint32_t)iw * (a.img8 ? 3u : 12u) : (uint32_t)(iw * CIN + 4 * q) * 4u;
-    tinfo[j] = (uint32_t)(xoff<CIN>(0, x, q >> 1) + 4 * (q & 1)) | ((uint32_t)(rr & 15) << 10) |
-               ((uint32_t)col_ok << 14) | ((uint32_t)(rr < R) << 15) | (tc << 16);
-  }
-  auto load_src = [&](int ih, int iw, bool col_ok) -> float4 {
-    if constexpr (STEM) {
-      const int pix = ih * W + iw;
-      const bool ok = col_ok && ih >= 0 && ih < H;
-      if (im8) {
-        const uint32_t off = ok ? (uint32_t)pix * 3u : 0x80000000u;
-        const uint32_t r = __builtin_amdgcn_raw_buffer_load_b8(rimg, off, 0, 0);
-        const uint32_t g = __builtin_amdgcn_raw_buffer_load_b8(rimg, off + 1u, 0, 0);
-        const uint32_t b = __builtin_amdgcn_raw_buffer_load_b8(rimg, off + 2u, 0, 0);
-        return make_float4(__builtin_bit_cast(float, r), __builtin_bit_cast(float, g), __builtin_bit_cast(float, b), 0.f);
-      }
-      const uint32_t off = ok ? (uint32_t)pix * 12u : 0x80000000u;
-      return make_float4(__builtin_bit_cast(float, __builtin_amdgcn_raw_buffer_load_b32(rimg, off, 0, 0)),
-                         __builtin_bit_cast(float, __builtin_amdgcn_raw_buffer_load_b32(rimg, off + 4u, 0, 0)),
-                         __builtin_bit_cast(float, __builtin_amdgcn_raw_buffer_load_b32(rimg, off + 8u, 0, 0)), 0.f);
-    } else {
-      const uint32_t off = col_ok ? (uint32_t)ih * ROWB + (uint32_t)(iw * CIN + 4 * q) * 4u : 0x80000000u;
-      return __builtin_bit_cast(float4, __builtin_amdgcn_raw_buffer_load_b128(rx, off, 0, 0));
-    }
-  };
-  auto img_px = [&](float4 v) -> float4 {
-    if (im8)
-      return make_float4((float)__builtin_bit_cast(uint32_t, v.x), (float)__builtin_bit_cast(uint32_t, v.y),
-                         (float)__builtin_bit_cast(uint32_t, v.z), 0.f);
-    return v;
-  };
-  auto load_task = [&](int r0, int j) -> float4 {
-    const uint32_t ti = tinfo[j];
-    const uint32_t off = (ti >> 14) & 1u ? (uint32_t)((r0 + (int)((ti >> 10) & 15)) * (STEM ? W * 3 * (im8 ? 1 : 4) : (int)ROWB)) + (ti >> 16)
-                                         : 0x80000000u;
-    if constexpr (STEM) {
-      if (im8) {
-        const uint32_t r = __builtin_amdgcn_raw_buffer_load_b8(rimg, off, 0, 0);
-        const uint32_t g = __builtin_amdgcn_raw_buffer_load_b8(rimg, off + 1u, 0, 0);
-        const uint32_t b = __builtin_amdgcn_raw_buffer_load_b8(rimg, off + 2u, 0, 0);
-        return make_float4(__builtin_bit_cast(float, r), __builtin_bit_cast(float, g), __builtin_bit_cast(float, b), 0.f);
-      }
-      return make_float4(__builtin_bit_cast(float, __builtin_amdgcn_raw_buffer_load_b32(rimg, off, 0, 0)),
-                         __builtin_bit_cast(float, __builtin_amdgcn_raw_buffer_load_b32(rimg, off + 4u, 0, 0)),
-                         __builtin_bit_cast(float, __builtin_amdgcn_raw_buffer_load_b32(rimg, off + 8u, 0, 0)), 0.f);
-    } else {
-      return __builtin_bit_cast(float4, __builtin_amdgcn_raw_buffer_load_b128(rx, off, 0, 0));
-    }
-  };
-  auto stage4 = [&](int o, bool in, float4 v, auto MASK_) {
-    constexpr bool MASK = decltype(MASK_)::value;
-    if constexpr (STEM) v = img_px(v);
-    float u[4];
-#pragma unroll
-    for (int c = 0; c < 4; ++c) {
-      if constexpr (STEM) {
-        float acc = v.x * bnw[c][0];
-        acc = fmaf(v.y, bnw[c][1], acc);
-        acc = fmaf(v.z, bnw[c][2], acc);
-        u[c] = acc + bnw[c][3];
-      } else {
-        u[c] = fmaf((&v.x)[c], bnw[c][0], bnw[c][1]);
-      }
-    }
-    float e[4];
-#pragma unroll
-    for (int c = 0; c < 4; ++c) e[c] = (!MASK || in) ? elu16(u[c]) : 0.0f;
-    rmax = fmaxf(rmax, amax4(e[0], e[1], e[2], e[3]));
-    f16x4 hv, lv;
-    split4(e[0], e[1], e[2], e[3], hv, lv);
-    *reinterpret_cast<f16x4*>(sx + o) = hv;
-    *reinterpret_cast<f16x4*>(sx + G::XPLANE + o) = lv;
-  };
-  auto stage_task = [&](int r0, int j, float4 v, auto MASK_) {
-    const uint32_t ti = tinfo[j];
-    if (((ti >> 14) & 3u) != 3u) return;
-    const int rr = (int)((ti >> 10) & 15);
-    uint32_t slot = (uint32_t)((r0 + 1) % G::XRING) + (uint32_t)rr;
-    slot = min(slot, slot - (uint32_t)G::XRING);
-    stage4((int)slot * G::XROW + (int)(ti & 1023), r0 + rr < H, v, MASK_);
-  };
-  for (int e = tid; e < 2 * G::XRING * G::XW * G::QPP; e += NT) {
-    const int pl = e / (G::XRING * G::XW * G::QPP), r = e - pl * (G::XRING * G::XW * G::QPP);
-    const int slot = r / (G::XW * G::QPP), x = (r / G::QPP) % G::XW, qq = r % G::QPP;
-    const int iw = w0 - 1 + x;
-    if (iw < 0 || iw >= W)
-      *reinterpret_cast<f16x4*>(sx + pl * G::XPLANE + xoff<CIN>(slot, x, qq >> 1) + 4 * (qq & 1)) = f16x4{};
-  }
-  const int n = lane & 31, nr = n >> 4, nc = n & 15;
-  int xco[3][G::KPT];
-#pragma unroll
-  for (int dx = 0; dx < 3; ++dx)
-#pragma unroll
-    for (int ks = 0; ks < G::KPT; ++ks) xco[dx][ks] = xoff<CIN>(0, nc + dx, G::KPT == 2 ? 2 * ks + h : h);
-
-  f16x8 w1h[G::PF], w1l[G::PF];
-  auto gemm1_issue = [&]() {
-#pragma unroll
-    for (int s = 0; s < G::PF; ++s) {
-      w1h[s] = w_frag(rw1h, s * 512, lofs);
-      w1l[s] = w_frag(rw1l, s * 512, lofs);
-    }
-  };
-  auto gemm1 = [&](int j0) -> f32x16 {
-    f32x16 acc;
-#pragma unroll
-    for (int i = 0; i < 16; ++i) acc[i] = 0.0f;
-    int xr[3];
-#pragma unroll
-    for (int dy = 0; dy < 3; ++dy) {
-      const uint32_t sl = (uint32_t)(j0 % G::XRING) + (uint32_t)(nr + dy);
-      xr[dy] = (int)min(sl, sl - (uint32_t)G::XRING) * G::XROW;
-    }
-    auto xo = [&](int s) {
-      const int tap = s / G::KPT, ks = s % G::KPT;
-      return xr[tap / 3] + xco[tap % 3][ks];
-    };
-    f16x8 nxh = *reinterpret_cast<const f16x8*>(sx + xo(0));
-    f16x8 nxl = *reinterpret_cast<const f16x8*>(sx + G::XPLANE + xo(0));
-#pragma unroll
-    for (int s = 0; s < G::KS1; ++s) {
-      const f16x8 bh = w1h[s % G::PF], bl = w1l[s % G::PF];
-      if (s + G::PF < G::KS1) {
-        w1h[s % G::PF] = w_frag(rw1h, (s + G::PF) * 512, lofs);
-        w1l[s % G::PF] = w_frag(rw1l, (s + G::PF) * 512, lofs);
-      }
-      const f16x8 xh = nxh, xl = nxl;
-      if (s + 1 < G::KS1) {
-        nxh = *reinterpret_cast<const f16x8*>(sx + xo(s + 1));
-        nxl = *reinterpret_cast<const f16x8*>(sx + G::XPLANE + xo(s + 1));
-      }
-      acc = __builtin_amdgcn_mfma_f32_32x32x16_f16(bl, xh, acc, 0, 0, 0);
-      acc = __builtin_amdgcn_mfma_f32_32x32x16_f16(bh, xl, acc, 0, 0, 0);
-      acc = __builtin_amdgcn_mfma_f32_32x32x16_f16(bh, xh, acc, 0, 0, 0);
-      __builtin_amdgcn_sched_barrier(0);
-    }
-    return acc;
-  };
-  auto t1_write = [&](int j0, const f32x16& acc) {
-    const int j = j0 + nr;
-    const uint32_t sl = (uint32_t)((j0 + 1) % G::TRING) + (uint32_t)nr;
-    const int slot = (int)min(sl, sl - (uint32_t)G::TRING);
-    if (j0 < H) {
-#pragma unroll
-      for (int jj = 0; jj < 4; ++jj) {
-        const int c0 = 8 * jj + 4 * h;
-        const float4 sv = spar[c0 / 4], cv = spar[C / 4 + c0 / 4];
-        float e[4];
-        e[0] = elu16(fmaf(acc[4 * jj + 0], sv.x, cv.x));
-        e[1] = elu16(fmaf(acc[4 * jj + 1], sv.y, cv.y));
-        e[2] = elu16(fmaf(acc[4 * jj + 2], sv.z, cv.z));
-        e[3] = elu16(fmaf(acc[4 * jj + 3], sv.w, cv.w));
-        rmax = fmaxf(rmax, amax4(e[0], e[1], e[2], e[3]));
-        f16x4 hv, lv;
-        split4(e[0], e[1], e[2], e[3], hv, lv);
-        const int o = toff<POOL>(slot, j, nc, jj) + 4 * h;
-        *reinterpret_cast<f16x4*>(st + o) = hv;
-        *reinterpret_cast<f16x4*>(st + G::TPLANE + o) = lv;
-      }
-    } else {
-#pragma unroll
-      for (int jj = 0; jj < 4; ++jj) {
-        const int o = toff<POOL>(slot, j, nc, jj) + 4 * h;
-        *reinterpret_cast<f16x4*>(st + o) = f16x4{};
-        *reinterpret_cast<f16x4*>(st + G::TPLANE + o) = f16x4{};
-      }
-    }
-  };
-
-  {
-    constexpr int T0 = 4 * G::XW * G::QPP;
-#pragma unroll
-    for (int j = 0; j < G::MAXT0; ++j) {
-      const int t = tid + j * NT;
-      const int px = t / G::QPP;
-      const int rr = px / G::XW, x = px - rr * G::XW;
-      const int ih = rr - 1, iw = w0 - 1 + x;
-      const bool col_ok = iw >= 0 && iw < W;
-      const float4 v = load_src(ih, iw, col_ok);
-      if (t < T0 && col_ok)
-        stage4(xoff<CIN>((ih + 1) % G::XRING, x, q >> 1) + 4 * (q & 1), ih >= 0, v, std::true_type{});
-    }
-    for (int e = tid; e < 2 * G::TROW / 8; e += NT)
-      *reinterpret_cast<f16x8*>(st + (e >= G::TROW / 8 ? G::TPLANE - G::TROW : 0) + 8 * e) = f16x8{};
-  }
-  __syncthreads();
-  if (wave == 0) {
-    gemm1_issue();
-    const f32x16 acc = gemm1(0);
-    t1_write(0, acc);
-  }
-  float4 preA[G::MAXT], preB[G::PD == 2 ? G::MAXT : 1];
-#pragma unroll
-  for (int j = 0; j < G::MAXT; ++j) preA[j] = load_task(3, j);
-  if constexpr (G::PD == 2) {
-#pragma unroll
-    for (int j = 0; j < G::MAXT; ++j) preB[j] = load_task(3 + R, j);
-  }
-  __syncthreads();
-
-  const int win = n >> 2;
-  const int sc_col = w0 + 2 * win;
-  float bsc = 0.0f;
-  if constexpr (POOL) bsc = a.bs[n];
-
-#if RBS_TRACE
-  unsigned long long tt[8];
-#endif
-  static_assert(G::NCHUNK % 2 == 0, "chunk pairs");
-  auto chunk = [&](const int k, float4* pre) {
-    RBS_T(0);
-    const int rx0 = R * k + 3;
-    const int j0 = R * k + 2 + 2 * wave;
-    const int o0 = R * k + 2 * wave;
-    if (k + 1 < G::NCHUNK) {
-#pragma unroll
-      for (int j = 0; j < G::MAXT; ++j) stage_task(rx0, j, pre[j], std::false_type{});
-    } else {
-#pragma unroll
-      for (int j = 0; j < G::MAXT; ++j) stage_task(rx0, j, pre[j], std::true_type{});
-    }
-    gemm1_issue();
-    RBS_T(1);
-    __syncthreads();
-    RBS_T(2);
-    {
-      const f32x16 acc = gemm1(j0);
-      RBS_T(3);
-      t1_write(j0, acc);
-    }
-    RBS_T(4);
-    const int pr = POOL ? (n & 3) >> 1 : nr;
-    const int pc = POOL ? 2 * (n >> 2) + (n & 1) : nc;
-    float4 rsd[POOL ? 1 : 4];
-    float4 scpx = make_float4(0.f, 0.f, 0.f, 0.f);
-    if constexpr (!POOL) {
-      const uint32_t off = w0 + pc < W ? (uint32_t)(o0 + pr) * ROWB + (uint32_t)((w0 + pc) * C + 4 * h) * 4u : 0x80000000u;
-#pragma unroll
-      for (int jj = 0; jj < 4; ++jj)
-        rsd[jj] = __builtin_bit_cast(float4, __builtin_amdgcn_raw_buffer_load_b128(rx, off, jj * 32, 0));
-    } else {
-      scpx = load_src(o0, sc_col, sc_col < W);
-    }
-    if (k + G::PD < G::NCHUNK) {
-#pragma unroll
-      for (int j = 0; j < G::MAXT; ++j) pre[j] = load_task(rx0 + G::PD * R, j);
-    }
-    __syncthreads();
-    RBS_T(5);
-    f32x16 acc;
-#pragma unroll
-    for (int i = 0; i < 16; ++i) acc[i] = 0.0f;
-    {
-      int tr[4], tj[4];
-#pragma unroll
-      for (int dy = 0; dy < 4; ++dy) {
-        tj[dy] = o0 + pr - 1 + dy;
-        const uint32_t sl = (uint32_t)(o0 % G::TRING) + (uint32_t)(pr + dy);
-        tr[dy] = (int)min(sl, sl - (uint32_t)G::TRING);
-      }
-      auto to = [&](int s) { return toff<POOL>(tr[s >> 1], tj[s >> 1], pc, 2 * (s & 1) + h); };
-      auto step2 = [&](f16x8 xh, f16x8 xl, f16x8 gh, f16x8 gl) {
-        if constexpr (POOL) {
-          acc = __builtin_amdgcn_mfma_f32_32x32x16_f16(xh, gl, acc, 0, 0, 0);
-          acc = __builtin_amdgcn_mfma_f32_32x32x16_f16(xl, gh, acc, 0, 0, 0);
-          acc = __builtin_amdgcn_mfma_f32_32x32x16_f16(xh, gh, acc, 0, 0, 0);
-        } else {
-          acc = __builtin_amdgcn_mfma_f32_32x32x16_f16(gl, xh, acc, 0, 0, 0);
-          acc = __builtin_amdgcn_mfma_f32_32x32x16_f16(gh, xl, acc, 0, 0, 0);
-          acc = __builtin_amdgcn_mfma_f32_32x32x16_f16(gh, xh, acc, 0, 0, 0);
-        }
-      };
-      if constexpr (G::W2L) {
-        f16x8 fxh[2], fxl[2], fgh[2], fgl[2];
-        auto fetch = [&](int s) {
-          fxh[s & 1] = *reinterpret_cast<const f16x8*>(st + to(s));
-          fxl[s & 1] = *reinterpret_cast<const f16x8*>(st + G::TPLANE + to(s));
-          fgh[s & 1] = *reinterpret_cast<const f16x8*>(sw2 + s * 512 + lofs);
-          fgl[s & 1] = *reinterpret_cast<const f16x8*>(sw2 + (G::KS2 + s) * 512 + lofs);
-        };
-        fetch(0);
-#pragma unroll
-        for (int s = 0; s < G::KS2; ++s) {
-          if (s + 1 < G::KS2) fetch(s + 1);
-          step2(fxh[s & 1], fxl[s & 1], fgh[s & 1], fgl[s & 1]);
-          if (s + 1 < G::KS2) pin_group<1, 4>(); else pin_group<1, 0>();
-        }
-      } else {
-        f16x8 nxh = *reinterpret_cast<const f16x8*>(st + to(0));
-        f16x8 nxl = *reinterpret_cast<const f16x8*>(st + G::TPLANE + to(0));
-#pragma unroll
-        for (int s = 0; s < G::KS2; ++s) {
-          const f16x8 xh = nxh, xl = nxl;
-          if (s + 1 < G::KS2) {
-            nxh = *reinterpret_cast<const f16x8*>(st + to(s + 1));
-            nxl = *reinterpret_cast<const f16x8*>(st + G::TPLANE + to(s + 1));
-          }
-          step2(xh, xl, w2h[s], w2l[s]);
-          __builtin_amdgcn_sched_barrier(0);
-        }
-      }
-    }
-    RBS_T(6);
-    if constexpr (!POOL) {
-      const int ow = w0 + pc, oh = o0 + pr;
-      if (ow < W) {
-#pragma unroll
-        for (int jj = 0; jj < 4; ++jj) {
-          const int c0 = 8 * jj + 4 * h;
-          const float4 b = spar[2 * C / 4 + c0 / 4];
-          const float4 r = rsd[jj];
-          const float4 v = make_float4(fmaf(acc[4 * jj + 0], a.u2, b.x) + r.x, fmaf(acc[4 * jj + 1], a.u2, b.y) + r.y,
-                                       fmaf(acc[4 * jj + 2], a.u2, b.z) + r.z, fmaf(acc[4 * jj + 3], a.u2, b.w) + r.w);
-          *reinterpret_cast<float4*>(a.y + (((int64_t)clip * H + oh) * W + ow) * C + c0) = v;
-        }
-      }
-    } else {
-      f32x16 sacc;
-#pragma unroll
-      for (int i = 0; i < 16; ++i) sacc[i] = 0.0f;
-      {
-        float o8[8];
-        const float4 px = img_px(scpx);
-#pragma unroll
-        for (int c = 0; c < 8; ++c) {
-          const float4 wv = spar[3 * C / 4 + 8 * h + c];
-          float s = px.x * wv.x;
-          s = fmaf(px.y, wv.y, s);
-          s = fmaf(px.z, wv.z, s);
-          o8[c] = sc_col < W ? 16.0f * (s + wv.w) : 0.0f;
-        }
-        rmax = fmaxf(rmax, fmaxf(amax4(o8[0], o8[1], o8[2], o8[3]), amax4(o8[4], o8[5], o8[6], o8[7])));
-        f16x4 h0, l0, h1, l1;
-        split4(o8[0], o8[1], o8[2], o8[3], h0, l0);
-        split4(o8[4], o8[5], o8[6], o8[7], h1, l1);
-        const f16x8 ah = {h0[0], h0[1], h0[2], h0[3], h1[0], h1[1], h1[2], h1[3]};
-        const f16x8 al = {l0[0], l0[1], l0[2], l0[3], l1[0], l1[1], l1[2], l1[3]};
-        sacc = __builtin_amdgcn_mfma_f32_32x32x16_f16(ah, wsl_, sacc, 0, 0, 0);
-        sacc = __builtin_amdgcn_mfma_f32_32x32x16_f16(al, wsh_, sacc, 0, 0, 0);
-        sacc = __builtin_amdgcn_mfma_f32_32x32x16_f16(ah, wsh_, sacc, 0, 0, 0);
-      }
-      constexpr int HP = H / 2, WP = (W + 1) / 2;
-      const int co = n;
-      const float b2 = sp[2 * C + co], bs = bsc;
-      const int prow = (R / 2) * k + wave;
-#pragma unroll
-      for (int jj = 0; jj < 4; ++jj) {
-        const int wdw = 2 * jj + h;
-        const int cc = w0 + 2 * wdw;
-        if (cc >= W) continue;
-        float m0 = fmaf(acc[4 * jj + 0], a.u2, b2);
-        float m1 = fmaf(acc[4 * jj + 1], a.u2, b2);
-        float m2 = fmaf(acc[4 * jj + 2], a.u2, b2);
-        float m3 = fmaf(acc[4 * jj + 3], a.u2, b2);
-        if (cc + 1 >= W) {
-          m1 = m0;
-          m3 = m2;
-        }
-        const float mx = fmaxf(fmaxf(m0, m1), fmaxf(m2, m3)) + fmaf(sacc[4 * jj], a.us, bs);
-        a.y[(((int64_t)clip * HP + prow) * WP + (w0 >> 1) + wdw) * C + co] = mx;
-      }
-    }
-    RBS_T(7);
-    RBS_TFLUSH();
-  };
-  if constexpr (G::PD == 2) {
-#pragma unroll 1
-    for (int k = 0; k < G::NCHUNK; k += 2) {
-      chunk(k, preA);
-      chunk(k + 1, preB);
-    }
-  } else {
-#pragma unroll 1
-    for (int k = 0; k < G::NCHUNK; ++k) chunk(k, preA);
-  }
-  if (!(rmax < SPLIT_MAX) && a.range_flag) *a.range_flag = 1;
-}
 
 template <int H, int W, int CIN, bool POOL, bool STEM>
 hipError_t launch(const ResBlkArgs& a, hipStream_t s) {
@@ -540,7 +25,7 @@
   return c == 32 && ((h == 128 && w == 151 && cin == 16 && pool) || (h == 64 && w == 76 && cin == 32 && !pool));
 }
 
-hipError_t rbs_launch(const ResBlkArgs& a, int cin, int c, bool pool, hipStream_t s) {
+hipError_t rbs_launch(const ResBlkArgs& a, int cin, int c, bool pool, bool w1_lds, hipStream_t s) {
   if (a.n == 0) return hipSuccess;
   if (!rbs_supported(a.h, a.w, cin, c, pool) || !a.y || !a.w1h || !a.w1l || !a.w2h || !a.w2l)
     return hipErrorInvalidValue;
@@ -550,5 +35,5 @@
     return hipErrorInvalidValue;
   }
   if (!a.x || a.x == a.y) return hipErrorInvalidValue;
-  return launch<64, 76, 32, false, false>(a, s);
+  return w1_lds ? rbs_w1l_launch(a, s) : launch<64, 76, 32, false, false>(a, s);
 }
diff --git a/mmla_audio_amd/csrc/rbs_body.h b/mmla_audio_amd/csrc/rbs_body.h
--- /dev/null
+++ b/mmla_audio_amd/csrc/rbs_body.h
@@ -0,0 +1,561 @@
+#pragma once
+#include "f16x3.h"
+#include "resblk.h"
+#if !defined(RBS_KERNEL) || !defined(RBS_W1L)
+#error "define RBS_KERNEL and RBS_W1L before including rbs_body.h"
+#endif
+
+namespace {
+
+constexpr int NT = 256;
+constexpr int TW = 16;
+constexpr int R = 8;
+constexpr int C = 32;
+#ifndef RBS_TRACE
+#define RBS_TRACE 0
+#endif
+#if RBS_TRACE
+__device__ unsigned long long rbs_trace_buf[2048 * 4 * 4 * 8];
+#define RBS_T(i) do { if (bid < 2048 && k >= 2 && k < 6) tt[i] = __builtin_amdgcn_s_memtime(); } while (0)
+#define RBS_TFLUSH() do { if (bid < 2048 && k >= 2 && k < 6 && lane == 0) { for (int i_ = 0; i_ < 8; ++i_) rbs_trace_buf[(((size_t)bid * 4 + wave) * 4 + (k - 2)) * 8 + i_] = tt[i_]; } } while (0)
+#else
+#define RBS_T(i) do { } while (0)
+#define RBS_TFLUSH() do { } while (0)
+#endif
+
+template <int H, int W, int CIN, bool POOL>
+struct SG {
+  static constexpr int XW = TW + 2;
+  static constexpr int XRING = R + 2, TRING = R + 3;
+  static constexpr int XROW = XW * CIN;
+  static constexpr int XPLANE = XRING * XROW;
+  static constexpr int TROW = TW * C;
+  static constexpr int TPLANE = TRING * TROW;
+  static constexpr int NCHUNK = H / R;
+  static constexpr int STRIPS = (W + TW - 1) / TW;
+  static constexpr int QPP = CIN / 4;
+  static constexpr int MAXT = (R * XW * QPP + NT - 1) / NT;
+  static constexpr int MAXT0 = (4 * XW * QPP + NT - 1) / NT;
+  static constexpr int KPT = CIN / 16;
+  static constexpr int KS1 = 9 * KPT, KS2 = 8;
+  static constexpr bool W2L = CIN == 16;
+  static constexpr int MINB = CIN == 16 ? 3 : 2;
+  static constexpr int PF = 3;
+  static constexpr int PD = CIN == 16 ? 1 : 2;
+  static_assert(H % R == 0, "geometry");
+  static_assert(NT % QPP == 0, "a thread's channel quad is fixed");
+  static_assert(XROW <= 1024 && W * CIN * 4 < 65536 && W * 12 < 65536, "staging task fields");
+};
+
+template <int CIN>
+MMLA_DEV int xoff(int slot, int x, int g) {
+  constexpr int XROW = (TW + 2) * CIN;
+  const int f = CIN == 32 ? ((x >> 1) & 3) : ((x >> 1) & 1);
+  return slot * XROW + x * CIN + 8 * (g ^ f);
+}
+template <bool POOL>
+MMLA_DEV int toff(int slot, int j, int c, int g) {
+  const int f = POOL ? (((c >> 2) ^ (2 * (j & 1))) & 3) : ((c >> 2) & 3);
+  return slot * (TW * C) + c * C + 8 * (g ^ f);
+}
+
+template <int H, int W, int CIN, bool POOL, bool STEM>
+__global__ void __launch_bounds__(NT, (SG<H, W, CIN, POOL>::MINB)) RBS_KERNEL(ResBlkArgs a) {
+  using G = SG<H, W, CIN, POOL>;
+  constexpr bool W1L = RBS_W1L;
+  static_assert(!STEM || (CIN == 16 && POOL), "the stem feeds block 1");
+  static_assert(POOL || CIN == C, "residual blocks keep their width");
+  static_assert(!W1L || G::MINB == 2, "LDS-resident GEMM 1 weights: two workgroups per CU");
+  constexpr int KS1L = W1L ? G::KS1 - 1 : 0;
+  static_assert(!W1L || 4 * (G::XPLANE + G::TPLANE + KS1L * 512) + 3 * C * 4 <= 160 * 1024 / 2, "LDS of two workgroups");
+  __shared__ __attribute__((aligned(16))) _Float16 sx[2 * G::XPLANE];
+  __shared__ __attribute__((aligned(16))) _Float16 st[2 * G::TPLANE];
+  __shared__ float4 spar[3 * C / 4 + (STEM ? 16 : 0)];
+  __shared__ __attribute__((aligned(16))) _Float16 sw2[G::W2L ? 2 * G::KS2 * 512 : 8];
+  __shared__ __attribute__((aligned(16))) _Float16 sw1[W1L ? 2 * KS1L * 512 : 8];
+
+  const int tid = threadIdx.x, lane = tid & 63;
+  const int wave = __builtin_amdgcn_readfirstlane(tid >> 6);
+  const int h = lane >> 5;
+  const uint32_t bid = xcd_block_id();
+  const int clip = (int)(bid / G::STRIPS);
+  const int w0 = (int)(bid - (uint32_t)clip * G::STRIPS) * TW;
+  const int lofs = lane * 8;
+  float rmax = 0.0f;
+
+  float* const sp = reinterpret_cast<float*>(spar);
+  if (tid < C) {
+    const float s2 = a.s2[tid];
+    sp[tid] = 16.0f * (s2 * a.u1);
+    sp[C + tid] = 16.0f * fmaf(a.b1[tid], s2, a.t2[tid]);
+    sp[2 * C + tid] = a.b2[tid];
+  }
+  if constexpr (STEM) {
+    if (tid < 64) {
+      const int co = tid >> 2, k = tid & 3;
+      sp[3 * C + tid] = k < 3 ? a.wst[k * a.ldst + co] : a.bst[co];
+    }
+  }
+  const __amdgpu_buffer_rsrc_t rw1h = w_rsrc(a.w1h), rw1l = w_rsrc(a.w1l);
+  f16x8 w2h[G::W2L ? 1 : G::KS2], w2l[G::W2L ? 1 : G::KS2];
+  if constexpr (G::W2L) {
+    for (int e = tid; e < 2 * G::KS2 * 64; e += NT) {
+      const int pl = e / (G::KS2 * 64), i = e - pl * (G::KS2 * 64);
+      *reinterpret_cast<f16x8*>(sw2 + 8 * e) = *reinterpret_cast<const f16x8*>((pl ? a.w2l : a.w2h) + 8 * i);
+    }
+  } else {
+    const __amdgpu_buffer_rsrc_t rw2h = w_rsrc(a.w2h), rw2l = w_rsrc(a.w2l);
+#pragma unroll
+    for (int s = 0; s < G::KS2; ++s) {
+      w2h[s] = w_frag(rw2h, s * 512, lofs);
+      w2l[s] = w_frag(rw2l, s * 512, lofs);
+    }
+  }
+  f16x8 w1th[W1L ? G::KS1 - KS1L : 1], w1tl[W1L ? G::KS1 - KS1L : 1];
+  if constexpr (W1L) {
+    for (int e = tid; e < 2 * KS1L * 64; e += NT) {
+      const int pl = e / (KS1L * 64), i = e - pl * (KS1L * 64);
+      *reinterpret_cast<f16x8*>(sw1 + 8 * e) = *reinterpret_cast<const f16x8*>((pl ? a.w1l : a.w1h) + 8 * i);
+    }
+#pragma unroll
+    for (int s = KS1L; s < G::KS1; ++s) {
+      w1th[s - KS1L] = w_frag(rw1h, s * 512, lofs);
+      w1tl[s - KS1L] = w_frag(rw1l, s * 512, lofs);
+    }
+  }
+  f16x8 wsh_, wsl_;
+  if constexpr (POOL) {
+    wsh_ = w_frag(w_rsrc(a.wsh), 0, lofs);
+    wsl_ = w_frag(w_rsrc(a.wsl), 0, lofs);
+  }
+  const int q = tid % G::QPP;
+  float bnw[4][4];
+  __syncthreads();
+#pragma unroll
+  for (int c = 0; c < 4; ++c) {
+    const float s16 = 16.0f * a.s1[4 * q + c], t16 = 16.0f * a.t1[4 * q + c];
+    if constexpr (STEM) {
+      const float4 v = spar[3 * C / 4 + 4 * q + c];
+      bnw[c][0] = s16 * v.x;
+      bnw[c][1] = s16 * v.y;
+      bnw[c][2] = s16 * v.z;
+      bnw[c][3] = fmaf(s16, v.w, t16);
+    } else {
+      bnw[c][0] = s16;
+      bnw[c][1] = t16;
+    }
+  }
+
+  constexpr uint32_t ROWB = STEM ? 0u : (uint32_t)W * CIN * 4;
+  const __amdgpu_buffer_rsrc_t rx = STEM ? w_rsrc(nullptr) :
+      __builtin_amdgcn_make_buffer_rsrc(const_cast<float*>(a.x) + (int64_t)clip * H * W * CIN, (short)0,
+                                        (int)(H * ROWB), 0x00020000);
+  const bool im8 = STEM && a.img8 != nullptr;
+  const __amdgpu_buffer_rsrc_t rimg = !STEM ? w_rsrc(nullptr) :
+      __builtin_amdgcn_make_buffer_rsrc(im8 ? (void*)(a.img8 + (int64_t)clip * H * W * 3)
+                                            : (void*)(a.imgf + (int64_t)clip * H * W * 3),
+                                        (short)0, (int)(H * W * 3 * (im8 ? 1 : 4)), 0x00020000);
+  uint32_t tinfo[G::MAXT];
+#pragma unroll
+  for (int j = 0; j < G::MAXT; ++j) {
+    const int t = tid + j * NT;
+    const int px = t / G::QPP;
+    const int rr = px / G::XW, x = px - rr * G::XW;
+    const int iw = w0 - 1 + x;
+    const bool col_ok = iw >= 0 && iw < W;
+    const uint32_t tc = !col_ok ? 0u : STEM ? (uint32_t)iw * (a.img8 ? 3u : 12u) : (uint32_t)(iw * CIN + 4 * q) * 4u;
+    tinfo[j] = (uint32_t)(xoff<CIN>(0, x, q >> 1) + 4 * (q & 1)) | ((uint32_t)(rr & 15) << 10) |
+               ((uint32_t)col_ok << 14) | ((uint32_t)(rr < R) << 15) | (tc << 16);
+  }
+  auto load_src = [&](int ih, int iw, bool col_ok) -> float4 {
+    if constexpr (STEM) {
+      const int pix = ih * W + iw;
+      const bool ok = col_ok && ih >= 0 && ih < H;
+      if (im8) {
+        const uint32_t off = ok ? (uint32_t)pix * 3u : 0x80000000u;
+        const uint32_t r = __builtin_amdgcn_raw_buffer_load_b8(rimg, off, 0, 0);
+        const uint32_t g = __builtin_amdgcn_raw_buffer_load_b8(rimg, off + 1u, 0, 0);
+        const uint32_t b = __builtin_amdgcn_raw_buffer_load_b8(rimg, off + 2u, 0, 0);
+        return make_float4(__builtin_bit_cast(float, r), __builtin_bit_cast(float, g), __builtin_bit_cast(float, b), 0.f);
+      }
+      const uint32_t off = ok ? (uint32_t)pix * 12u : 0x80000000u;
+      return make_float4(__builtin_bit_cast(float, __builtin_amdgcn_raw_buffer_load_b32(rimg, off, 0, 0)),
+                         __builtin_bit_cast(float, __builtin_amdgcn_raw_buffer_load_b32(rimg, off + 4u, 0, 0)),
+                         __builtin_bit_cast(float, __builtin_amdgcn_raw_buffer_load_b32(rimg, off + 8u, 0, 0)), 0.f);
+    } else {
+      const uint32_t off = col_ok ? (uint32_t)ih * ROWB + (uint32_t)(iw * CIN + 4 * q) * 4u : 0x80000000u;
+      return __builtin_bit_cast(float4, __builtin_amdgcn_raw_buffer_load_b128(rx, off, 0, 0));
+    }
+  };
+  auto img_px = [&](float4 v) -> float4 {
+    if (im8)
+      return make_float4((float)__builtin_bit_cast(uint32_t, v.x), (float)__builtin_bit_cast(uint32_t, v.y),
+                         (float)__builtin_bit_cast(uint32_t, v.z), 0.f);
+    return v;
+  };
+  auto load_task = [&](int r0, int j) -> float4 {
+    const uint32_t ti = tinfo[j];
+    const uint32_t off = (ti >> 14) & 1u ? (uint32_t)((r0 + (int)((ti >> 10) & 15)) * (STEM ? W * 3 * (im8 ? 1 : 4) : (int)ROWB)) + (ti >> 16)
+                                         : 0x80000000u;
+    if constexpr (STEM) {
+      if (im8) {
+        const uint32_t r = __builtin_amdgcn_raw_buffer_load_b8(rimg, off, 0, 0);
+        const uint32_t g = __builtin_amdgcn_raw_buffer_load_b8(rimg, off + 1u, 0, 0);
+        const uint32_t b = __builtin_amdgcn_raw_buffer_load_b8(rimg, off + 2u, 0, 0);
+        return make_float4(__builtin_bit_cast(float, r), __builtin_bit_cast(float, g), __builtin_bit_cast(float, b), 0.f);
+      }
+      return make_float4(__builtin_bit_cast(float, __builtin_amdgcn_raw_buffer_load_b32(rimg, off, 0, 0)),
+                         __builtin_bit_cast(float, __builtin_amdgcn_raw_buffer_load_b32(rimg, off + 4u, 0, 0)),
+                         __builtin_bit_cast(float, __builtin_amdgcn_raw_buffer_load_b32(rimg, off + 8u, 0, 0)), 0.f);
+    } else {
+      return __builtin_bit_cast(float4, __builtin_amdgcn_raw_buffer_load_b128(rx, off, 0, 0));
+    }
+  };
+  auto stage4 = [&](int o, bool in, float4 v, auto MASK_) {
+    constexpr bool MASK = decltype(MASK_)::value;
+    if constexpr (STEM) v = img_px(v);
+    float u[4];
+#pragma unroll
+    for (int c = 0; c < 4; ++c) {
+      if constexpr (STEM) {
+        float acc = v.x * bnw[c][0];
+        acc = fmaf(v.y, bnw[c][1], acc);
+        acc = fmaf(v.z, bnw[c][2], acc);
+        u[c] = acc + bnw[c][3];
+      } else {
+        u[c] = fmaf((&v.x)[c], bnw[c][0], bnw[c][1]);
+      }
+    }
+    float e[4];
+#pragma unroll
+    for (int c = 0; c < 4; ++c) e[c] = (!MASK || in) ? elu16(u[c]) : 0.0f;
+    rmax = fmaxf(rmax, amax4(e[0], e[1], e[2], e[3]));
+    f16x4 hv, lv;
+    split4(e[0], e[1], e[2], e[3], hv, lv);
+    *reinterpret_cast<f16x4*>(sx + o) = hv;
+    *reinterpret_cast<f16x4*>(sx + G::XPLANE + o) = lv;
+  };
+  auto stage_task = [&](int r0, int j, float4 v, auto MASK_) {
+    const uint32_t ti = tinfo[j];
+    if (((ti >> 14) & 3u) != 3u) return;
+    const int rr = (int)((ti >> 10) & 15);
+    uint32_t slot = (uint32_t)((r0 + 1) % G::XRING) + (uint32_t)rr;
+    slot = min(slot, slot - (uint32_t)G::XRING);
+    stage4((int)slot * G::XROW + (int)(ti & 1023), r0 + rr < H, v, MASK_);
+  };
+  for (int e = tid; e < 2 * G::XRING * G::XW * G::QPP; e += NT) {
+    const int pl = e / (G::XRING * G::XW * G::QPP), r = e - pl * (G::XRING * G::XW * G::QPP);
+    const int slot = r / (G::XW * G::QPP), x = (r / G::QPP) % G::XW, qq = r % G::QPP;
+    const int iw = w0 - 1 + x;
+    if (iw < 0 || iw >= W)
+      *reinterpret_cast<f16x4*>(sx + pl * G::XPLANE + xoff<CIN>(slot, x, qq >> 1) + 4 * (qq & 1)) = f16x4{};
+  }
+  const int n = lane & 31, nr = n >> 4, nc = n & 15;
+  int xco[3][G::KPT];
+#pragma unroll
+  for (int dx = 0; dx < 3; ++dx)
+#pragma unroll
+    for (int ks = 0; ks < G::KPT; ++ks) xco[dx][ks] = xoff<CIN>(0, nc + dx, G::KPT == 2 ? 2 * ks + h : h);
+
+  f16x8 w1h[W1L ? 1 : G::PF], w1l[W1L ? 1 : G::PF];
+  auto gemm1_issue = [&]() {
+    if constexpr (!W1L) {
+#pragma unroll
+      for (int s = 0; s < G::PF; ++s) {
+        w1h[s] = w_frag(rw1h, s * 512, lofs);
+        w1l[s] = w_frag(rw1l, s * 512, lofs);
+      }
+    }
+  };
+  auto gemm1 = [&](int j0) -> f32x16 {
+    f32x16 acc;
+#pragma unroll
+    for (int i = 0; i < 16; ++i) acc[i] = 0.0f;
+    int xr[3];
+#pragma unroll
+    for (int dy = 0; dy < 3; ++dy) {
+      const uint32_t sl = (uint32_t)(j0 % G::XRING) + (uint32_t)(nr + dy);
+      xr[dy] = (int)min(sl, sl - (uint32_t)G::XRING) * G::XROW;
+    }
+    auto xo = [&](int s) {
+      const int tap = s / G::KPT, ks = s % G::KPT;
+      return xr[tap / 3] + xco[tap % 3][ks];
+    };
+    f16x8 nxh = *reinterpret_cast<const f16x8*>(sx + xo(0));
+    f16x8 nxl = *reinterpret_cast<const f16x8*>(sx + G::XPLANE + xo(0));
+    f16x8 nbh, nbl;
+    if constexpr (W1L) {
+      nbh = *reinterpret_cast<const f16x8*>(sw1 + lofs);
+      nbl = *reinterpret_cast<const f16x8*>(sw1 + KS1L * 512 + lofs);
+    }
+#pragma unroll
+    for (int s = 0; s < G::KS1; ++s) {
+      f16x8 bh, bl;
+      if constexpr (W1L) {
+        bh = s < KS1L ? nbh : w1th[s < KS1L ? 0 : s - KS1L];
+        bl = s < KS1L ? nbl : w1tl[s < KS1L ? 0 : s - KS1L];
+        if (s + 1 < KS1L) {
+          nbh = *reinterpret_cast<const f16x8*>(sw1 + (s + 1) * 512 + lofs);
+          nbl = *reinterpret_cast<const f16x8*>(sw1 + (KS1L + s + 1) * 512 + lofs);
+        }
+      } else {
+        bh = w1h[s % G::PF];
+        bl = w1l[s % G::PF];
+        if (s + G::PF < G::KS1) {
+          w1h[s % G::PF] = w_frag(rw1h, (s + G::PF) * 512, lofs);
+          w1l[s % G::PF] = w_frag(rw1l, (s + G::PF) * 512, lofs);
+        }
+      }
+      const f16x8 xh = nxh, xl = nxl;
+      if (s + 1 < G::KS1) {
+        nxh = *reinterpret_cast<const f16x8*>(sx + xo(s + 1));
+        nxl = *reinterpret_cast<const f16x8*>(sx + G::XPLANE + xo(s + 1));
+      }
+      acc = __builtin_amdgcn_mfma_f32_32x32x16_f16(bl, xh, acc, 0, 0, 0);
+      acc = __builtin_amdgcn_mfma_f32_32x32x16_f16(bh, xl, acc, 0, 0, 0);
+      acc = __builtin_amdgcn_mfma_f32_32x32x16_f16(bh, xh, acc, 0, 0, 0);
+      __builtin_amdgcn_sched_barrier(0);
+    }
+    return acc;
+  };
+  auto t1_write = [&](int j0, const f32x16& acc) {
+    const int j = j0 + nr;
+    const uint32_t sl = (uint32_t)((j0 + 1) % G::TRING) + (uint32_t)nr;
+    const int slot = (int)min(sl, sl - (uint32_t)G::TRING);
+    if (j0 < H) {
+#pragma unroll
+      for (int jj = 0; jj < 4; ++jj) {
+        const int c0 = 8 * jj + 4 * h;
+        const float4 sv = spar[c0 / 4], cv = spar[C / 4 + c0 / 4];
+        float e[4];
+        e[0] = elu16(fmaf(acc[4 * jj + 0], sv.x, cv.x));
+        e[1] = elu16(fmaf(acc[4 * jj + 1], sv.y, cv.y));
+        e[2] = elu16(fmaf(acc[4 * jj + 2], sv.z, cv.z));
+        e[3] = elu16(fmaf(acc[4 * jj + 3], sv.w, cv.w));
+        rmax = fmaxf(rmax, amax4(e[0], e[1], e[2], e[3]));
+        f16x4 hv, lv;
+        split4(e[0], e[1], e[2], e[3], hv, lv);
+        const int o = toff<POOL>(slot, j, nc, jj) + 4 * h;
+        *reinterpret_cast<f16x4*>(st + o) = hv;
+        *reinterpret_cast<f16x4*>(st + G::TPLANE + o) = lv;
+      }
+    } else {
+#pragma unroll
+      for (int jj = 0; jj < 4; ++jj) {
+        const int o = toff<POOL>(slot, j, nc, jj) + 4 * h;
+        *reinterpret_cast<f16x4*>(st + o) = f16x4{};
+        *reinterpret_cast<f16x4*>(st + G::TPLANE + o) = f16x4{};
+      }
+    }
+  };
+
+  {
+    constexpr int T0 = 4 * G::XW * G::QPP;
+#pragma unroll
+    for (int j = 0; j < G::MAXT0; ++j) {
+      const int t = tid + j * NT;
+      const int px = t / G::QPP;
+      const int rr = px / G::XW, x = px - rr * G::XW;
+      const int ih = rr - 1, iw = w0 - 1 + x;
+      const bool col_ok = iw >= 0 && iw < W;
+      const float4 v = load_src(ih, iw, col_ok);
+      if (t < T0 && col_ok)
+        stage4(xoff<CIN>((ih + 1) % G::XRING, x, q >> 1) + 4 * (q & 1), ih >= 0, v, std::true_type{});
+    }
+    for (int e = tid; e < 2 * G::TROW / 8; e += NT)
+      *reinterpret_cast<f16x8*>(st + (e >= G::TROW / 8 ? G::TPLANE - G::TROW : 0) + 8 * e) = f16x8{};
+  }
+  __syncthreads();
+  if (wave == 0) {
+    gemm1_issue();
+    const f32x16 acc = gemm1(0);
+    t1_write(0, acc);
+  }
+  float4 preA[G::MAXT], preB[G::PD == 2 ? G::MAXT : 1];
+#pragma unroll
+  for (int j = 0; j < G::MAXT; ++j) preA[j] = load_task(3, j);
+  if constexpr (G::PD == 2) {
+#pragma unroll
+    for (int j = 0; j < G::MAXT; ++j) preB[j] = load_task(3 + R, j);
+  }
+  __syncthreads();
+
+  const int win = n >> 2;
+  const int sc_col = w0 + 2 * win;
+  float bsc = 0.0f;
+  if constexpr (POOL) bsc = a.bs[n];
+
+#if RBS_TRACE
+  unsigned long long tt[8];
+#endif
+  static_assert(G::NCHUNK % 2 == 0, "chunk pairs");
+  auto chunk = [&](const int k, float4* pre) {
+    RBS_T(0);
+    const int rx0 = R * k + 3;
+    const int j0 = R * k + 2 + 2 * wave;
+    const int o0 = R * k + 2 * wave;
+    if (k + 1 < G::NCHUNK) {
+#pragma unroll
+      for (int j = 0; j < G::MAXT; ++j) stage_task(rx0, j, pre[j], std::false_type{});
+    } else {
+#pragma unroll
+      for (int j = 0; j < G::MAXT; ++j) stage_task(rx0, j, pre[j], std::true_type{});
+    }
+    gemm1_issue();
+    RBS_T(1);
+    __syncthreads();
+    RBS_T(2);
+    {
+      const f32x16 acc = gemm1(j0);
+      RBS_T(3);
+      t1_write(j0, acc);
+    }
+    RBS_T(4);
+    const int pr = POOL ? (n & 3) >> 1 : nr;
+    const int pc = POOL ? 2 * (n >> 2) + (n & 1) : nc;
+    float4 rsd[POOL ? 1 : 4];
+    float4 scpx = make_float4(0.f, 0.f, 0.f, 0.f);
+    if constexpr (!POOL) {
+      const uint32_t off = w0 + pc < W ? (uint32_t)(o0 + pr) * ROWB + (uint32_t)((w0 + pc) * C + 4 * h) * 4u : 0x80000000u;
+#pragma unroll
+      for (int jj = 0; jj < 4; ++jj)
+        rsd[jj] = __builtin_bit_cast(float4, __builtin_amdgcn_raw_buffer_load_b128(rx, off, jj * 32, 0));
+    } else {
+      scpx = load_src(o0, sc_col, sc_col < W);
+    }
+    if (k + G::PD < G::NCHUNK) {
+#pragma unroll
+      for (int j = 0; j < G::MAXT; ++j) pre[j] = load_task(rx0 + G::PD * R, j);
+    }
+    __syncthreads();
+    RBS_T(5);
+    f32x16 acc;
+#pragma unroll
+    for (int i = 0; i < 16; ++i) acc[i] = 0.0f;
+    {
+      int tr[4], tj[4];
+#pragma unroll
+      for (int dy = 0; dy < 4; ++dy) {
+        tj[dy] = o0 + pr - 1 + dy;
+        const uint32_t sl = (uint32_t)(o0 % G::TRING) + (uint32_t)(pr + dy);
+        tr[dy] = (int)min(sl, sl - (uint32_t)G::TRING);
+      }
+      auto to = [&](int s) { return toff<POOL>(tr[s >> 1], tj[s >> 1], pc, 2 * (s & 1) + h); };
+      auto step2 = [&](f16x8 xh, f16x8 xl, f16x8 gh, f16x8 gl) {
+        if constexpr (POOL) {
+          acc = __builtin_amdgcn_mfma_f32_32x32x16_f16(xh, gl, acc, 0, 0, 0);
+          acc = __builtin_amdgcn_mfma_f32_32x32x16_f16(xl, gh, acc, 0, 0, 0);
+          acc = __builtin_amdgcn_mfma_f32_32x32x16_f16(xh, gh, acc, 0, 0, 0);
+        } else {
+          acc = __builtin_amdgcn_mfma_f32_32x32x16_f16(gl, xh, acc, 0, 0, 0);
+          acc = __builtin_amdgcn_mfma_f32_32x32x16_f16(gh, xl, acc, 0, 0, 0);
+          acc = __builtin_amdgcn_mfma_f32_32x32x16_f16(gh, xh, acc, 0, 0, 0);
+        }
+      };
+      if constexpr (G::W2L) {
+        f16x8 fxh[2], fxl[2], fgh[2], fgl[2];
+        auto fetch = [&](int s) {
+          fxh[s & 1] = *reinterpret_cast<const f16x8*>(st + to(s));
+          fxl[s & 1] = *reinterpret_cast<const f16x8*>(st + G::TPLANE + to(s));
+          fgh[s & 1] = *reinterpret_cast<const f16x8*>(sw2 + s * 512 + lofs);
+          fgl[s & 1] = *reinterpret_cast<const f16x8*>(sw2 + (G::KS2 + s) * 512 + lofs);
+        };
+        fetch(0);
+#pragma unroll
+        for (int s = 0; s < G::KS2; ++s) {
+          if (s + 1 < G::KS2) fetch(s + 1);
+          step2(fxh[s & 1], fxl[s & 1], fgh[s & 1], fgl[s & 1]);
+          if (s + 1 < G::KS2) pin_group<1, 4>(); else pin_group<1, 0>();
+        }
+      } else {
+        f16x8 nxh = *reinterpret_cast<const f16x8*>(st + to(0));
+        f16x8 nxl = *reinterpret_cast<const f16x8*>(st + G::TPLANE + to(0));
+#pragma unroll
+        for (int s = 0; s < G::KS2; ++s) {
+          const f16x8 xh = nxh, xl = nxl;
+          if (s + 1 < G::KS2) {
+            nxh = *reinterpret_cast<const f16x8*>(st + to(s + 1));
+            nxl = *reinterpret_cast<const f16x8*>(st + G::TPLANE + to(s + 1));
+          }
+          step2(xh, xl, w2h[s], w2l[s]);
+          __builtin_amdgcn_sched_barrier(0);
+        }
+      }
+    }
+    RBS_T(6);
+    if constexpr (!POOL) {
+      const int ow = w0 + pc, oh = o0 + pr;
+      if (ow < W) {
+#pragma unroll
+        for (int jj = 0; jj < 4; ++jj) {
+          const int c0 = 8 * jj + 4 * h;
+          const float4 b = spar[2 * C / 4 + c0 / 4];
+          const float4 r = rsd[jj];
+          const float4 v = make_float4(fmaf(acc[4 * jj + 0], a.u2, b.x) + r.x, fmaf(acc[4 * jj + 1], a.u2, b.y) + r.y,
+                                       fmaf(acc[4 * jj + 2], a.u2, b.z) + r.z, fmaf(acc[4 * jj + 3], a.u2, b.w) + r.w);
+          *reinterpret_cast<float4*>(a.y + (((int64_t)clip * H + oh) * W + ow) * C + c0) = v;
+        }
+      }
+    } else {
+      f32x16 sacc;
+#pragma unroll
+      for (int i = 0; i < 16; ++i) sacc[i] = 0.0f;
+      {
+        float o8[8];
+        const float4 px = img_px(scpx);
+#pragma unroll
+        for (int c = 0; c < 8; ++c) {
+          const float4 wv = spar[3 * C / 4 + 8 * h + c];
+          float s = px.x * wv.x;
+          s = fmaf(px.y, wv.y, s);
+          s = fmaf(px.z, wv.z, s);
+          o8[c] = sc_col < W ? 16.0f * (s + wv.w) : 0.0f;
+        }
+        rmax = fmaxf(rmax, fmaxf(amax4(o8[0], o8[1], o8[2], o8[3]), amax4(o8[4], o8[5], o8[6], o8[7])));
+        f16x4 h0, l0, h1, l1;
+        split4(o8[0], o8[1], o8[2], o8[3], h0, l0);
+        split4(o8[4], o8[5], o8[6], o8[7], h1, l1);
+        const f16x8 ah = {h0[0], h0[1], h0[2], h0[3], h1[0], h1[1], h1[2], h1[3]};
+        const f16x8 al = {l0[0], l0[1], l0[2], l0[3], l1[0], l1[1], l1[2], l1[3]};
+        sacc = __builtin_amdgcn_mfma_f32_32x32x16_f16(ah, wsl_, sacc, 0, 0, 0);
+        sacc = __builtin_amdgcn_mfma_f32_32x32x16_f16(al, wsh_, sacc, 0, 0, 0);
+        sacc = __builtin_amdgcn_mfma_f32_32x32x16_f16(ah, wsh_, sacc, 0, 0, 0);
+      }
+      constexpr int HP = H / 2, WP = (W + 1) / 2;
+      const int co = n;
+      const float b2 = sp[2 * C + co], bs = bsc;
+      const int prow = (R / 2) * k + wave;
+#pragma unroll
+      for (int jj = 0; jj < 4; ++jj) {
+        const int wdw = 2 * jj + h;
+        const int cc = w0 + 2 * wdw;
+        if (cc >= W) continue;
+        float m0 = fmaf(acc[4 * jj + 0], a.u2, b2);
+        float m1 = fmaf(acc[4 * jj + 1], a.u2, b2);
+        float m2 = fmaf(acc[4 * jj + 2], a.u2, b2);
+        float m3 = fmaf(acc[4 * jj + 3], a.u2, b2);
+        if (cc + 1 >= W) {
+          m1 = m0;
+          m3 = m2;
+        }
+        const float mx = fmaxf(fmaxf(m0, m1), fmaxf(m2, m3)) + fmaf(sacc[4 * jj], a.us, bs);
+        a.y[(((int64_t)clip * HP + prow) * WP + (w0 >> 1) + wdw) * C + co] = mx;
+      }
+    }
+    RBS_T(7);
+    RBS_TFLUSH();
+  };
+  if constexpr (G::PD == 2) {
+#pragma unroll 1
+    for (int k = 0; k < G::NCHUNK; k += 2) {
+      chunk(k, preA);
+      chunk(k + 1, preB);
+    }
+  } else {
+#pragma unroll 1
+    for (int k = 0; k < G::NCHUNK; ++k) chunk(k, preA);
+  }
+  if (!(rmax < SPLIT_MAX) && a.range_flag) *a.range_flag = 1;
+}
+
+}
diff --git a/mmla_audio_amd/csrc/rbs_w1l.hip b/mmla_audio_amd/csrc/rbs_w1l.hip
--- /dev/null
+++ b/mmla_audio_amd/csrc/rbs_w1l.hip
@@ -0,0 +1,17 @@
+#define RBS_KERNEL rbs_w1l_kernel
+#define RBS_W1L true
+#include "rbs_body.h"
+
+#if RBS_TRACE
+extern "C" int mmla_debug_rbs_w1l_trace(unsigned long long* out) {
+  return hipMemcpyFromSymbol(out, HIP_SYMBOL(rbs_trace_buf), sizeof(rbs_trace_buf)) == hipSuccess ? 0 : -2;
+}
+#endif
+
+hipError_t rbs_w1l_launch(const ResBlkArgs& a, hipStream_t s) {
+  using G = SG<64, 76, 32, false>;
+  const int64_t blocks = (int64_t)a.n * G::STRIPS;
+  if (blocks > 0x7fffffffLL) return hipErrorInvalidValue;
+  hipLaunchKernelGGL((rbs_w1l_kernel<64, 76, 32, false, false>), dim3((unsigned)blocks), dim3(NT), 0, s, a);
+  return hipGetLastError();
+}
diff --git a/mmla_audio_amd/csrc/resblk.h b/mmla_audio_amd/csrc/resblk.h
--- a/mmla_audio_amd/csrc/resblk.h
+++ b/mmla_audio_amd/csrc/resblk.h
@@ -36,4 +36,5 @@
                           uint16_t* lo, bool frag, float wscale);
 
 bool rbs_supported(int h, int w, int cin, int c, bool pool);
-hipError_t rbs_launch(const ResBlkArgs& a, int cin, int c, bool pool, hipStream_t stream);
+hipError_t rbs_launch(const ResBlkArgs& a, int cin, int c, bool pool, bool w1_lds, hipStream_t stream);
+hipError_t rbs_w1l_launch(const ResBlkArgs& a, hipStream_t stream);
```

After: 172,700, median of 6. 1.02x the previous value.
